# SerezD/gen_adversarial

Hardware: AMD Instinct MI355X
Metric: purified images/sec (attack+encode+decode) (higher is better)
Workload: dtype f32 storage; contractions as 3x bf16 MFMA (hi/lo split), fp32 accumulate; 1 GPU; configs[1]: NVAE purify + VGG-11, 64x64, PGD-Linf step (fwd + input-grad), bs 256 images/GPU x EoT 32 = 8192 defender rows per step, alphas ours_cosine_no_preprocessing_ids.yaml x0.7, assumed NVAE config (C=32, 3x8 groups, 20 latents); images_per_gpu=256, eot=32, rows_per_gpu=8192, chunk_rows=1024, streams=2, parallelism=image-sharded x1

## Files before the change

### gen_adversarial_amd/_lib.py

```python
from __future__ import annotations

import ctypes as C
import os

import torch

_HERE = os.path.dirname(os.path.abspath(__file__))
LIB_PATH = os.environ.get('GA_OPS_LIB') or os.path.join(_HERE, 'libga_ops.so')

GA_ACT_NONE, GA_ACT_SILU, GA_ACT_ELU, GA_ACT_RELU, GA_ACT_LRELU, GA_ACT_FLRELU = 0, 1, 2, 3, 4, 5
GA_CONV_ADDEND_RELU, GA_CONV_ADDEND_PRE_DACT, GA_CONV_PRO_PRELU, GA_CONV_DACT_PRELU = 1, 2, 4, 8
(GA_OP_CONV, GA_OP_DWCONV5, GA_OP_REDUCE, GA_OP_SE_EXCITE, GA_OP_SE_APPLY, GA_OP_BILINEAR_BWD, GA_OP_SAMPLER,
 GA_OP_DML, GA_OP_MAXPOOL, GA_OP_IMAGE_IO, GA_OP_AXPBY, GA_OP_BLUR, GA_OP_REP_SUM, GA_OP_INTERLEAVE2,
 GA_OP_MAXPOOL3S2, GA_OP_AVGPOOL_ACT, GA_OP_GCONV, GA_OP_PRELU, GA_OP_UNARY, GA_OP_MODOUT, GA_OP_UP2_BLUR, GA_OP_PIXELNORM,
 GA_OP_LATENT_MIX, GA_OP_POOL_DENORM, GA_OP_ATTN, GA_OP_LAYERNORM, GA_OP_RESIZE2_CROP, GA_OP_DEC_CELL, GA_OP_AVAE, GA_OP_DEC_CELL_HALO) = range(1, 31)
GA_AVAE_ADAIN, GA_AVAE_AVGPOOL, GA_AVAE_PIXELNORM, GA_AVAE_SAMPLE = 0, 1, 2, 3
ABI_VERSION = 8
ERRORS = {0: 'GA_OK', -1: 'GA_E_BADARG', -2: 'GA_E_ALIGN', -3: 'GA_E_UNSUPPORTED', -4: 'GA_E_LAUNCH'}

fp = C.c_void_p
i32 = C.c_int
f32 = C.c_float


class ConvDesc(C.Structure):
    _fields_ = [('x', fp), ('ldx', i32), ('x2', fp), ('ldx2', i32), ('w', fp), ('bias', fp),
                ('pro_scale', fp), ('pro_shift', fp), ('addend', fp), ('ldadd', i32),
                ('addend2', fp), ('ldadd2', i32), ('dact_x', fp), ('lddact', i32),
                ('dact_scale', fp), ('dact_shift', fp), ('y', fp), ('ldy', i32),
                ('N', i32), ('Hi', i32), ('Wi', i32), ('C1', i32), ('C2', i32),
                ('Ho', i32), ('Wo', i32), ('Cout', i32),
                ('KH', i32), ('KW', i32), ('sn', i32), ('sd', i32), ('pad', i32),
                ('pro_act', i32), ('pro_per_row', i32), ('dact_act', i32), ('addend_bcast_n', i32), ('tile', i32),
                ('splits', i32), ('ws', fp), ('ws_floats', C.c_long),
                ('x_bytes', C.c_uint), ('x2_bytes', C.c_uint), ('w_bytes', C.c_uint), ('dact_rep', i32),
                ('w_hi', fp), ('w_lo', fp), ('addend_rep', i32), ('flags', i32), ('w_frag', fp)]


class DwDesc(C.Structure):
    _fields_ = [('x', fp), ('w', fp), ('bias', fp), ('dact_x', fp), ('y', fp),
                ('N', i32), ('H', i32), ('W', i32), ('C', i32),
                ('pro_act', i32), ('dact_act', i32), ('up2', i32), ('pool2', i32), ('act_rep', i32), ('_reserved', i32)]


class ReduceDesc(C.Structure):
    _fields_ = [('a', fp), ('b', fp), ('out', fp), ('N', i32), ('P', i32), ('C', i32), ('scale', f32),
                ('ws', fp), ('ws_floats', C.c_long), ('gate', fp), ('skip', fp), ('scaled', fp), ('a_src', fp), ('a_w', fp)]


class SeExciteDesc(C.Structure):
    _fields_ = [('m', fp), ('w1', fp), ('b1', fp), ('w2', fp), ('b2', fp), ('hid', fp), ('gate', fp),
                ('dgate', fp), ('pro_scale', fp), ('pro_shift', fp),
                ('N', i32), ('C', i32), ('Hd', i32), ('P', i32), ('res_scale', f32), ('backward', i32),
                ('t', fp), ('dout', fp), ('skip', fp), ('out', fp), ('act_rep', i32), ('_reserved', i32)]


class SeApplyDesc(C.Structure):
    _fields_ = [('skip', fp), ('t', fp), ('gate', fp), ('out', fp),
                ('N', i32), ('H', i32), ('W', i32), ('C', i32), ('skip_mode', i32), ('res_scale', f32)]


class BilinearBwdDesc(C.Structure):
    _fields_ = [('dhigh', fp), ('dlow', fp), ('N', i32), ('h', i32), ('w', i32), ('C', i32), ('accumulate', i32)]


class SamplerDesc(C.Structure):
    _fields_ = [('mu_q', fp), ('ldq', i32), ('p', fp), ('ldp', i32), ('eps', fp), ('eps_nchw', i32),
                ('z', fp), ('dz', fp), ('dmu_q', fp), ('dp', fp),
                ('N', i32), ('h', i32), ('w', i32), ('NL', i32),
                ('alpha', f32), ('one_minus_alpha', f32), ('temp', f32), ('backward', i32),
                ('q_rep', i32), ('dmu_q_rows', fp), ('ldz', i32), ('act_rep', i32), ('mode', i32), ('_reserved', i32),
                ('alpha_rows', fp), ('alpha_ld', i32), ('alpha_col', i32)]


class DmlDesc(C.Structure):
    _fields_ = [('logits', fp), ('ld', i32), ('nmix', i32), ('img_nchw', fp), ('img_nhwc', fp),
                ('dimg_nhwc', fp), ('dimg_nchw', fp), ('dlogits', fp),
                ('N', i32), ('H', i32), ('W', i32), ('backward', i32), ('ld_img', i32), ('act_rep', i32)]


class MaxpoolDesc(C.Structure):
    _fields_ = [('x', fp), ('y', fp), ('dy', fp), ('dx', fp), ('N', i32), ('H', i32), ('W', i32), ('C', i32),
                ('backward', i32), ('act_rep', i32)]


class ImageIoDesc(C.Structure):
    _fields_ = [('x_nchw', fp), ('noise_nchw', fp), ('noise_coef', fp), ('y_nhwc', fp), ('dy_nhwc', fp),
                ('dx_nchw', fp), ('N', i32), ('C', i32), ('H', i32), ('W', i32), ('rep', i32), ('backward', i32),
                ('ld', i32), ('s2d', i32), ('cot_rep', i32), ('_reserved', i32)]


class AxpbyDesc(C.Structure):
    _fields_ = [('x', fp), ('y', fp), ('n', C.c_long), ('alpha', f32), ('beta', f32)]


class BlurDesc(C.Structure):
    _fields_ = [('x', fp), ('y', fp), ('taps', fp), ('planes', i32), ('H', i32), ('W', i32), ('k', i32), ('backward', i32),
                ('radius', i32), ('tmp', fp)]


class RepSumDesc(C.Structure):
    _fields_ = [('x', fp), ('y', fp), ('rows', C.c_long), ('inner', C.c_long), ('rep', i32), ('accumulate', i32)]


class Interleave2Desc(C.Structure):
    _fields_ = [('s', fp * 4), ('y', fp), ('dact_x', fp), ('dact_scale', fp), ('dact_shift', fp), ('addend', fp),
                ('addend2', fp), ('N', i32), ('H', i32), ('W', i32), ('C', i32), ('dact_act', i32), ('dact_prelu', i32),
                ('lds', i32), ('dact_rep', i32)]


class Maxpool3s2Desc(C.Structure):
    _fields_ = [('x', fp), ('y', fp), ('dy', fp), ('dx', fp), ('N', i32), ('H', i32), ('W', i32), ('C', i32),
                ('backward', i32)]


class AvgpoolActDesc(C.Structure):
    _fields_ = [('x', fp), ('y', fp), ('dy', fp), ('dx', fp), ('N', i32), ('P', i32), ('C', i32), ('act', i32),
                ('backward', i32), ('_reserved', i32)]


class GconvDesc(C.Structure):
    _fields_ = [('x', fp), ('w', fp), ('bias', fp), ('dact_x', fp), ('y', fp),
                ('N', i32), ('Hi', i32), ('Wi', i32), ('Ho', i32), ('Wo', i32), ('C', i32), ('cg', i32),
                ('KH', i32), ('KW', i32), ('stride', i32), ('pad', i32), ('pro_act', i32), ('dact_act', i32), ('_reserved', i32)]


class PreluDesc(C.Structure):
    _fields_ = [('x', fp), ('slope', fp), ('y', fp), ('dy', fp), ('dx', fp), ('rows', C.c_long), ('C', i32), ('backward', i32)]


class UnaryDesc(C.Structure):
    _fields_ = [('x', fp), ('g', fp), ('y', fp), ('n', C.c_long), ('mode', i32), ('eps', f32)]


class ModoutDesc(C.Structure):
    _fields_ = [('t', fp), ('scale', fp), ('add', fp), ('out', fp), ('dout', fp), ('dt', fp),
                ('N', i32), ('P', i32), ('C', i32), ('act', i32), ('backward', i32), ('W', i32), ('dt_planes', fp * 4),
                ('ld_planes', i32), ('_reserved2', i32), ('red', fp), ('ws', fp), ('ws_floats', C.c_long), ('t_planes', fp * 4)]


class Up2BlurDesc(C.Structure):
    _fields_ = [('lo_in', fp), ('hi', fp), ('hi_in', fp), ('lo', fp), ('N', i32), ('H', i32), ('W', i32), ('C', i32),
                ('backward', i32), ('_reserved', i32)]


class PixelnormDesc(C.Structure):
    _fields_ = [('x', fp), ('y', fp), ('rows', C.c_long), ('C', i32)]


class LatentMixDesc(C.Structure):
    _fields_ = [('codes', fp), ('avg', fp), ('styles', fp), ('alpha', fp), ('out', fp), ('dout', fp), ('dcodes', fp),
                ('R', i32), ('J', i32), ('D', i32), ('backward', i32), ('rep', i32), ('alpha_ld', i32)]


class PoolDenormDesc(C.Structure):
    _fields_ = [('x', fp), ('y', fp), ('dy', fp), ('dx', fp), ('N', i32), ('H', i32), ('W', i32), ('k', i32), ('ld', i32),
                ('backward', i32), ('dy_nchw', fp), ('band', i32), ('_reserved', i32)]


class AttnDesc(C.Structure):
    _fields_ = [('q', fp), ('k', fp), ('v', fp), ('out', fp), ('p', fp), ('dout', fp), ('ds', fp), ('dq', fp), ('dk', fp), ('dv', fp),
                ('ldq', i32), ('ldk', i32), ('ldv', i32), ('ldo', i32), ('lddq', i32), ('lddk', i32), ('lddv', i32),
                ('N', i32), ('Tq', i32), ('Tk', i32), ('heads', i32), ('dh', i32), ('scale', f32), ('backward', i32)]


class LayernormDesc(C.Structure):
    _fields_ = [('a', fp), ('b', fp), ('gamma', fp), ('beta', fp), ('y', fp), ('stats', fp), ('dy', fp), ('dx', fp),
                ('rows', C.c_long), ('C', i32), ('eps', f32), ('backward', i32), ('accumulate', i32)]


class Resize2CropDesc(C.Structure):
    _fields_ = [('x', fp), ('y', fp), ('dy', fp), ('dx', fp), ('N', i32), ('H', i32), ('W', i32), ('C', i32), ('crop', i32),
                ('backward', i32), ('accumulate', i32), ('_reserved', i32)]


class DecCellDesc(C.Structure):
    _fields_ = [('x', fp), ('w1_hi', fp), ('w1_lo', fp), ('b1', fp), ('wd', fp), ('wd_bwd', fp), ('bd', fp),
                ('w2_hi', fp), ('w2_lo', fp), ('b2', fp), ('dout', fp), ('pro_scale', fp), ('pro_shift', fp), ('y', fp),
                ('N', i32), ('H', i32), ('W', i32), ('C', i32), ('Hd', i32), ('backward', i32), ('act_rep', i32), ('variant', i32)]


class DecCellHaloDesc(C.Structure):
    _fields_ = [('x', fp), ('w1_hi', fp), ('w1_lo', fp), ('b1', fp), ('wd', fp), ('wd_bwd', fp), ('bd', fp),
                ('w2_hi', fp), ('w2_lo', fp), ('b2', fp), ('w1t_hi', fp), ('w1t_lo', fp), ('dout', fp), ('pro_scale', fp), ('pro_shift', fp),
                ('addend', fp), ('addend2', fp), ('y', fp),
                ('N', i32), ('H', i32), ('W', i32), ('Cin', i32), ('Cout', i32), ('Hd', i32), ('backward', i32), ('up', i32)]


class AvaeDesc(C.Structure):
    _fields_ = [('x', fp), ('a', fp), ('b', fp), ('c', fp), ('s', fp), ('dy', fp), ('y', fp), ('y2', fp),
                ('mode', i32), ('backward', i32), ('N', i32), ('P', i32), ('C', i32), ('k', i32), ('H', i32), ('W', i32),
                ('f0', f32), ('_reserved', i32)]


class _OpUnion(C.Union):
    _fields_ = [('conv', ConvDesc), ('dw', DwDesc), ('red', ReduceDesc), ('se', SeExciteDesc), ('app', SeApplyDesc),
                ('bil', BilinearBwdDesc), ('smp', SamplerDesc), ('dml', DmlDesc), ('mp', MaxpoolDesc),
                ('io', ImageIoDesc), ('ax', AxpbyDesc), ('blur', BlurDesc), ('rs', RepSumDesc), ('il', Interleave2Desc),
                ('mp3', Maxpool3s2Desc), ('ap', AvgpoolActDesc), ('gc', GconvDesc), ('pr', PreluDesc), ('un', UnaryDesc), ('mo', ModoutDesc), ('ub', Up2BlurDesc), ('lm', LatentMixDesc),
                ('pd', PoolDenormDesc), ('at', AttnDesc), ('ln', LayernormDesc), ('rc', Resize2CropDesc), ('dc', DecCellDesc), ('pn', PixelnormDesc), ('av', AvaeDesc), ('dh', DecCellHaloDesc)]


class Op(C.Structure):
    _fields_ = [('kind', i32), ('_pad', i32), ('u', _OpUnion)]


_KIND_FIELD = {GA_OP_CONV: 'conv', GA_OP_DWCONV5: 'dw', GA_OP_REDUCE: 'red', GA_OP_SE_EXCITE: 'se',
               GA_OP_SE_APPLY: 'app', GA_OP_BILINEAR_BWD: 'bil', GA_OP_SAMPLER: 'smp', GA_OP_DML: 'dml',
               GA_OP_MAXPOOL: 'mp', GA_OP_IMAGE_IO: 'io', GA_OP_AXPBY: 'ax', GA_OP_BLUR: 'blur', GA_OP_REP_SUM: 'rs',
               GA_OP_INTERLEAVE2: 'il', GA_OP_MAXPOOL3S2: 'mp3', GA_OP_AVGPOOL_ACT: 'ap', GA_OP_GCONV: 'gc', GA_OP_PRELU: 'pr', GA_OP_UNARY: 'un', GA_OP_MODOUT: 'mo', GA_OP_UP2_BLUR: 'ub', GA_OP_PIXELNORM: 'pn',
               GA_OP_LATENT_MIX: 'lm', GA_OP_POOL_DENORM: 'pd', GA_OP_ATTN: 'at', GA_OP_LAYERNORM: 'ln', GA_OP_RESIZE2_CROP: 'rc', GA_OP_DEC_CELL: 'dc', GA_OP_AVAE: 'av', GA_OP_DEC_CELL_HALO: 'dh'}
_DESC_KIND = {ConvDesc: GA_OP_CONV, DwDesc: GA_OP_DWCONV5, ReduceDesc: GA_OP_REDUCE, SeExciteDesc: GA_OP_SE_EXCITE,
              SeApplyDesc: GA_OP_SE_APPLY, BilinearBwdDesc: GA_OP_BILINEAR_BWD, SamplerDesc: GA_OP_SAMPLER,
              DmlDesc: GA_OP_DML, MaxpoolDesc: GA_OP_MAXPOOL, ImageIoDesc: GA_OP_IMAGE_IO, AxpbyDesc: GA_OP_AXPBY,
              BlurDesc: GA_OP_BLUR, RepSumDesc: GA_OP_REP_SUM, Interleave2Desc: GA_OP_INTERLEAVE2,
              Maxpool3s2Desc: GA_OP_MAXPOOL3S2, AvgpoolActDesc: GA_OP_AVGPOOL_ACT, GconvDesc: GA_OP_GCONV,
              PreluDesc: GA_OP_PRELU, UnaryDesc: GA_OP_UNARY, ModoutDesc: GA_OP_MODOUT, Up2BlurDesc: GA_OP_UP2_BLUR,
              PixelnormDesc: GA_OP_PIXELNORM, LatentMixDesc: GA_OP_LATENT_MIX, PoolDenormDesc: GA_OP_POOL_DENORM,
              AttnDesc: GA_OP_ATTN, LayernormDesc: GA_OP_LAYERNORM, Resize2CropDesc: GA_OP_RESIZE2_CROP, DecCellDesc: GA_OP_DEC_CELL, AvaeDesc: GA_OP_AVAE, DecCellHaloDesc: GA_OP_DEC_CELL_HALO}

EXPORTS = ['ga_conv2d', 'ga_dwconv5', 'ga_rowchan_reduce', 'ga_se_excite', 'ga_se_apply', 'ga_bilinear_up2_bwd',
           'ga_sampler_mix', 'ga_dml_mean', 'ga_maxpool2', 'ga_image_io', 'ga_axpby', 'ga_plan_run', 'ga_plan_time',
           'ga_plan_profile', 'ga_split_bf16', 'ga_gauss_blur', 'ga_rep_sum', 'ga_interleave2', 'ga_maxpool3s2', 'ga_avgpool_act', 'ga_gconv', 'ga_prelu', 'ga_unary', 'ga_modout', 'ga_up2_blur', 'ga_pixelnorm', 'ga_latent_mix', 'ga_pool_denorm', 'ga_attn', 'ga_layernorm', 'ga_resize2_crop', 'ga_dec_cell', 'ga_dec_cell_supported', 'ga_dec_cell_halo', 'ga_dec_cell_halo_supported', 'ga_avae', 'ga_microbench_hbm_copy', 'ga_microbench_mfma_bf16', 'ga_microbench_mfma_bf16_shape', 'ga_graph_capture', 'ga_graph_launch', 'ga_graph_destroy',
           'ga_last_hip_error', 'ga_abi_version', 'ga_sizeof_op', 'ga_debug_set_conv_row_limit']


def _load():
    if not os.path.exists(LIB_PATH):
        raise ImportError(f'{LIB_PATH} is missing: build it with `python -c "import __graft_entry__ as g; g.build()"` '
                          f'or `make -C gen_adversarial_amd/csrc` — there is no CPU fallback on the product path')
    lib = C.CDLL(LIB_PATH)
    for n, d in (('ga_conv2d', ConvDesc), ('ga_dwconv5', DwDesc), ('ga_rowchan_reduce', ReduceDesc),
                 ('ga_se_excite', SeExciteDesc), ('ga_se_apply', SeApplyDesc), ('ga_bilinear_up2_bwd', BilinearBwdDesc),
                 ('ga_sampler_mix', SamplerDesc), ('ga_dml_mean', DmlDesc), ('ga_maxpool2', MaxpoolDesc),
                 ('ga_image_io', ImageIoDesc), ('ga_gauss_blur', BlurDesc), ('ga_interleave2', Interleave2Desc),
                 ('ga_maxpool3s2', Maxpool3s2Desc), ('ga_avgpool_act', AvgpoolActDesc), ('ga_gconv', GconvDesc), ('ga_prelu', PreluDesc),
                 ('ga_unary', UnaryDesc), ('ga_modout', ModoutDesc), ('ga_up2_blur', Up2BlurDesc),
                 ('ga_latent_mix', LatentMixDesc), ('ga_pool_denorm', PoolDenormDesc), ('ga_attn', AttnDesc),
                 ('ga_layernorm', LayernormDesc), ('ga_resize2_crop', Resize2CropDesc), ('ga_dec_cell', DecCellDesc), ('ga_avae', AvaeDesc), ('ga_dec_cell_halo', DecCellHaloDesc)):
        f = getattr(lib, n)
        f.argtypes = [C.POINTER(d), C.c_void_p]
        f.restype = C.c_int
    lib.ga_axpby.argtypes = [fp, fp, C.c_long, f32, f32, C.c_void_p]
    lib.ga_axpby.restype = C.c_int
    lib.ga_plan_run.argtypes = [C.POINTER(Op), C.c_int, C.c_void_p, C.POINTER(C.c_int)]
    lib.ga_plan_run.restype = C.c_int
    lib.ga_plan_time.argtypes = [C.POINTER(Op), C.c_int, C.c_void_p, C.c_int, C.POINTER(f32), C.POINTER(f32),
                                 C.POINTER(C.c_long)]
    lib.ga_plan_time.restype = C.c_int
    lib.ga_plan_profile.argtypes = [C.POINTER(Op), C.c_int, C.c_void_p, C.POINTER(f32)]
    lib.ga_plan_profile.restype = C.c_int
    lib.ga_rep_sum.argtypes = [fp, fp, C.c_long, C.c_long, C.c_int, C.c_int, C.c_void_p]
    lib.ga_rep_sum.restype = C.c_int
    lib.ga_pixelnorm.argtypes = [fp, fp, C.c_long, C.c_int, C.c_void_p]
    lib.ga_pixelnorm.restype = C.c_int
    lib.ga_graph_capture.argtypes = [C.POINTER(Op), C.c_int, C.c_void_p, C.POINTER(C.c_void_p)]
    lib.ga_graph_capture.restype = C.c_int
    lib.ga_graph_launch.argtypes = [C.c_void_p, C.c_void_p]
    lib.ga_graph_launch.restype = C.c_int
    lib.ga_graph_destroy.argtypes = [C.c_void_p]
    lib.ga_graph_destroy.restype = C.c_int
    lib.ga_split_bf16.argtypes = [fp, fp, fp, C.c_long, C.c_void_p]
    lib.ga_split_bf16.restype = C.c_int
    lib.ga_last_hip_error.restype = C.c_char_p
    lib.ga_abi_version.restype = C.c_int
    lib.ga_sizeof_op.restype = C.c_ulong
    lib.ga_debug_set_conv_row_limit.restype = C.c_long
    lib.ga_dec_cell_supported.argtypes = [C.c_int] * 5
    lib.ga_dec_cell_supported.restype = C.c_int
    lib.ga_dec_cell_halo_supported.argtypes = [C.c_int] * 5
    lib.ga_dec_cell_halo_supported.restype = C.c_int
    lib.ga_debug_set_conv_row_limit.argtypes = [C.c_long]
    lib.ga_microbench_hbm_copy.argtypes = [fp, fp, C.c_long, C.c_void_p]
    lib.ga_microbench_hbm_copy.restype = C.c_int
    lib.ga_microbench_mfma_bf16.argtypes = [fp, C.c_int, C.c_int, C.c_void_p]
    lib.ga_microbench_mfma_bf16.restype = C.c_int
    lib.ga_microbench_mfma_bf16_shape.argtypes = [fp, C.c_int, C.c_int, C.c_int, C.c_void_p]
    lib.ga_microbench_mfma_bf16_shape.restype = C.c_int
    if lib.ga_abi_version() != ABI_VERSION:
        raise ImportError(f'ABI mismatch: {LIB_PATH} reports GA_ABI_VERSION {lib.ga_abi_version()}, the binding is written for '
                          f'{ABI_VERSION}: rebuild with `make -C gen_adversarial_amd/csrc`')
    if lib.ga_sizeof_op() != C.sizeof(Op):
        raise ImportError(f'ABI mismatch: library ga_op is {lib.ga_sizeof_op()} bytes, binding is {C.sizeof(Op)}')
    return lib


lib = _load()


class GaError(RuntimeError):
    pass


def check(rc: int, what: str = ''):
    if rc != 0:
        extra = f' ({lib.ga_last_hip_error().decode()})' if rc == -4 else ''
        raise GaError(f'{what}: {ERRORS.get(rc, rc)}{extra}')


def make_op(desc) -> Op:
    op = Op()
    op.kind = _DESC_KIND[type(desc)]
    setattr(op.u, _KIND_FIELD[op.kind], desc)
    return op


_DIRECT = {ConvDesc: 'ga_conv2d', DwDesc: 'ga_dwconv5', ReduceDesc: 'ga_rowchan_reduce', SeExciteDesc: 'ga_se_excite',
           SeApplyDesc: 'ga_se_apply', BilinearBwdDesc: 'ga_bilinear_up2_bwd', SamplerDesc: 'ga_sampler_mix',
           DmlDesc: 'ga_dml_mean', MaxpoolDesc: 'ga_maxpool2', ImageIoDesc: 'ga_image_io', BlurDesc: 'ga_gauss_blur',
           Interleave2Desc: 'ga_interleave2', Maxpool3s2Desc: 'ga_maxpool3s2', AvgpoolActDesc: 'ga_avgpool_act',
           GconvDesc: 'ga_gconv', PreluDesc: 'ga_prelu', UnaryDesc: 'ga_unary', ModoutDesc: 'ga_modout', Up2BlurDesc: 'ga_up2_blur',
           LatentMixDesc: 'ga_latent_mix', PoolDenormDesc: 'ga_pool_denorm', AttnDesc: 'ga_attn', LayernormDesc: 'ga_layernorm',
           Resize2CropDesc: 'ga_resize2_crop', DecCellDesc: 'ga_dec_cell', AvaeDesc: 'ga_avae', DecCellHaloDesc: 'ga_dec_cell_halo'}


def run(desc, stream: int = 0):
    if isinstance(desc, AxpbyDesc):
        check(lib.ga_axpby(desc.x, desc.y, desc.n, desc.alpha, desc.beta, stream), 'ga_axpby')
        return
    if isinstance(desc, PixelnormDesc):
        check(lib.ga_pixelnorm(desc.x, desc.y, desc.rows, desc.C, stream), 'ga_pixelnorm')
        return
    if isinstance(desc, RepSumDesc):
        check(lib.ga_rep_sum(desc.x, desc.y, desc.rows, desc.inner, desc.rep, desc.accumulate, stream), 'ga_rep_sum')
        return
    name = _DIRECT[type(desc)]
    check(getattr(lib, name)(C.byref(desc), stream), name)


class Plan:

    def __init__(self):
        self.descs = []
        self.names = []
        self._arr = None

    def add(self, desc, name: str = ''):
        self.descs.append(desc)
        self.names.append(name)
        self._arr = None

    def finalize(self):
        arr = (Op * len(self.descs))()
        for i, d in enumerate(self.descs):
            arr[i] = make_op(d)
        self._arr = arr
        return self

    def __len__(self):
        return len(self.descs)

    def run(self, stream: int = 0, start: int = 0, end: int = None):
        if self._arr is None:
            self.finalize()
        end = len(self.descs) if end is None else end
        if end <= start:
            return
        failed = C.c_int(-1)
        first = C.cast(C.byref(self._arr, start * C.sizeof(Op)), C.POINTER(Op))
        rc = lib.ga_plan_run(first, end - start, stream, C.byref(failed))
        if rc != 0:
            check(rc, f'plan op #{start + failed.value} ({self.names[start + failed.value]})')

    def capture(self, stream: int):
        if self._arr is None:
            self.finalize()
        h = C.c_void_p()
        check(lib.ga_graph_capture(self._arr, len(self.descs), stream, C.byref(h)), 'ga_graph_capture')
        return h

    @staticmethod
    def launch_graph(handle, stream: int):
        check(lib.ga_graph_launch(handle, stream), 'ga_graph_launch')

    @staticmethod
    def destroy_graph(handle):
        lib.ga_graph_destroy(handle)

    def profile(self, stream: int = 0):
        if self._arr is None:
            self.finalize()
        out = (f32 * len(self.descs))()
        check(lib.ga_plan_profile(self._arr, len(self.descs), stream, out), 'ga_plan_profile')
        return list(out)

    def time(self, stream: int = 0, iters: int = 1, per_conv: bool = False):
        if self._arr is None:
            self.finalize()
        total, conv, nconv = f32(0), f32(0), C.c_long(0)
        rc = lib.ga_plan_time(self._arr, len(self.descs), stream, iters, C.byref(total),
                              C.byref(conv) if per_conv else None, C.byref(nconv) if per_conv else None)
        check(rc, 'ga_plan_time')
        return total.value, conv.value, nconv.value
```

### gen_adversarial_amd/csrc/conv_epilogue.h

```cpp
#pragma once
#include "ga_common.h"

namespace ga {

__device__ __forceinline__ size_t dact_row(const ga_conv_desc& d, const size_t m, const int HoWo) {
    if (d.dact_rep <= 1) return m;
    const size_t n = m / (size_t)HoWo;
    return (n / (size_t)d.dact_rep) * (size_t)HoWo + (m - n * (size_t)HoWo);
}

__device__ __forceinline__ void epilogue4(const ga_conv_desc& d, const int m, const int co, floatx4 v, const int HoWo) {
    if (d.bias) v += *reinterpret_cast<const floatx4*>(d.bias + co);
    if ((d.flags & GA_CONV_ADDEND_PRE_DACT) && d.addend) v += *reinterpret_cast<const floatx4*>(d.addend + (size_t)m * d.ldadd + co);
    if (d.dact_x) {
        floatx4 u = *reinterpret_cast<const floatx4*>(d.dact_x + dact_row(d, (size_t)m, HoWo) * d.lddact + co);
        floatx4 ds = {1.f, 1.f, 1.f, 1.f};
        if (d.flags & GA_CONV_DACT_PRELU) {
            ds = *reinterpret_cast<const floatx4*>(d.dact_scale + co);
#pragma unroll
            for (int e = 0; e < 4; ++e) v[e] *= u[e] > 0.f ? 1.f : ds[e];
        } else {
            if (d.dact_scale) {
                ds = *reinterpret_cast<const floatx4*>(d.dact_scale + co);
                u = u * ds + *reinterpret_cast<const floatx4*>(d.dact_shift + co);
            }
#pragma unroll
            for (int e = 0; e < 4; ++e) v[e] *= act_bwd_fast(u[e], d.dact_act) * ds[e];
        }
    }
    if (d.addend && !(d.flags & GA_CONV_ADDEND_PRE_DACT)) {
        size_t am = d.addend_bcast_n ? (size_t)(m % HoWo) : (size_t)m;
        if (d.addend_rep > 1) am = (size_t)((m / HoWo) / d.addend_rep) * HoWo + (m % HoWo);
        floatx4 a = *reinterpret_cast<const floatx4*>(d.addend + am * d.ldadd + co);
        if (d.flags & GA_CONV_ADDEND_RELU) { for (int e = 0; e < 4; ++e) a[e] = fmaxf(a[e], 0.f); }
        v += a;
    }
    if (d.addend2) v += *reinterpret_cast<const floatx4*>(d.addend2 + (size_t)m * d.ldadd2 + co);
    *reinterpret_cast<floatx4*>(d.y + (size_t)m * d.ldy + co) = v;
}

__device__ __forceinline__ void epilogue1(const ga_conv_desc& d, const int m, const int co, float v, const int HoWo) {
    if (d.bias) v += d.bias[co];
    if ((d.flags & GA_CONV_ADDEND_PRE_DACT) && d.addend) v += d.addend[(size_t)m * d.ldadd + co];
    if (d.dact_x) {
        float ds = 1.f, db = 0.f;
        if (d.dact_scale) { ds = d.dact_scale[co]; db = d.dact_shift[co]; }
        if (d.flags & GA_CONV_DACT_PRELU) {
            v *= d.dact_x[dact_row(d, (size_t)m, HoWo) * d.lddact + co] > 0.f ? 1.f : ds;
        } else {
            const float u = d.dact_x[dact_row(d, (size_t)m, HoWo) * d.lddact + co] * ds + db;
            v *= act_bwd_fast(u, d.dact_act) * ds;
        }
    }
    if (d.addend && !(d.flags & GA_CONV_ADDEND_PRE_DACT)) {
        size_t am = d.addend_bcast_n ? (size_t)(m % HoWo) : (size_t)m;
        if (d.addend_rep > 1) am = (size_t)((m / HoWo) / d.addend_rep) * HoWo + (m % HoWo);
        const float a = d.addend[am * d.ldadd + co];
        v += (d.flags & GA_CONV_ADDEND_RELU) ? fmaxf(a, 0.f) : a;
    }
    if (d.addend2) v += d.addend2[(size_t)m * d.ldadd2 + co];
    d.y[(size_t)m * d.ldy + co] = v;
}


template <int TM, int TN, class F>
__device__ __forceinline__ void acc_walk(floatx16 (&acc)[TM][TN], const int lane, F&& f) {
    const int lrow = lane & 31, lh = lane >> 5;
#pragma unroll
    for (int i = 0; i < TM; ++i)
#pragma unroll
        for (int j = 0; j < TN; ++j)
#pragma unroll
            for (int r = 0; r < 16; ++r) f(i * 32 + (r & 3) + 8 * (r >> 2) + 4 * lh, j * 32 + lrow, acc[i][j][r]);
}
template <int TM2, int TN2, class F>
__device__ __forceinline__ void acc_walk(floatx4 (&acc)[TM2][TN2], const int lane, F&& f) {
    const int lc = lane & 15, lq = lane >> 4;
#pragma unroll
    for (int i = 0; i < TM2; ++i)
#pragma unroll
        for (int j = 0; j < TN2; ++j)
#pragma unroll
            for (int r = 0; r < 4; ++r) f(i * 16 + 4 * lq + r, j * 16 + lc, acc[i][j][r]);
}

template <int WM, int WN, int TM, int TN, class ACC>
__device__ __forceinline__ void conv_epilogue(const ga_conv_desc& d, ACC& acc, float* smem, const int m0,
                                              const int n0, const int M, const int vec_out, const int splits, const int split,
                                              const int tw_shift = 31, const int row_stride = 0) {
    const int tw_mask = (int)((1u << tw_shift) - 1u);
    auto mrow = [&](const int r) __attribute__((always_inline)) { return m0 + (r >> tw_shift) * row_stride + (r & tw_mask); };
    constexpr int BM = WM * TM * 32, BN = WN * TN * 32;
    constexpr int LDC = BN + 4;
    const int tid = threadIdx.x, lane = tid & 63, wave = tid >> 6;
    const int wm = wave / WN, wn = wave % WN;
    const int HoWo = d.Ho * d.Wo;
    float* ws = splits > 1 ? d.ws + (size_t)split * M * d.Cout : nullptr;
    if (vec_out) {
        float* Cs = smem;
        constexpr int QL = BN / 4;
        constexpr int ROWS = 256 / QL;
        constexpr int NB = (BM / ROWS) < 4 ? (BM / ROWS) : 4;
        constexpr int NIT = BM / (ROWS * NB);
        static_assert(NIT * ROWS * NB == BM, "whole batches");
        const int q = tid % QL, rr = tid / QL;
        const int co = n0 + 4 * q;
        const bool mine = co < d.Cout;
        floatx4 u[1][NB], a1[1][NB], a2[1][NB];
        auto issue = [&](const int set, const int rb0) __attribute__((always_inline)) {
#pragma unroll
            for (int k = 0; k < NB; ++k) {
                const int r = rb0 + k * ROWS;
                const int mr = mrow(r);
                const bool ok = mr < M;
                if (d.dact_x) {
                    const size_t m = ok ? dact_row(d, (size_t)mr, HoWo) : 0;
                    u[set][k] = *reinterpret_cast<const floatx4*>(d.dact_x + m * d.lddact + co);
                }
                if (d.addend) {
                    size_t m = ok ? (size_t)mr : 0;
                    if (d.addend_bcast_n) m = m % HoWo;
                    if (d.addend_rep > 1) m = ((m / HoWo) / d.addend_rep) * HoWo + (m % HoWo);
                    a1[set][k] = *reinterpret_cast<const floatx4*>(d.addend + m * d.ldadd + co);
                }
                if (d.addend2) {
                    const size_t m = ok ? (size_t)mr : 0;
                    a2[set][k] = *reinterpret_cast<const floatx4*>(d.addend2 + m * d.ldadd2 + co);
                }
            }
        };
        floatx4 bias4 = {0.f, 0.f, 0.f, 0.f}, ds4 = {1.f, 1.f, 1.f, 1.f}, dt4 = {0.f, 0.f, 0.f, 0.f};
        if (mine && !ws) {
            if (d.bias) bias4 = *reinterpret_cast<const floatx4*>(d.bias + co);
            if (d.dact_x && d.dact_scale) {
                ds4 = *reinterpret_cast<const floatx4*>(d.dact_scale + co);
                dt4 = *reinterpret_cast<const floatx4*>(d.dact_shift + co);
            }
        }
        acc_walk(acc, lane, [&](const int row, const int col, const float v) {
            Cs[(wm * TM * 32 + row) * LDC + wn * TN * 32 + col] = v;
        });
        __syncthreads();
        if (mine) {
#pragma unroll 1
            for (int it = 0; it < NIT; ++it) {
                const int rb0 = rr + it * ROWS * NB, set = 0;
                floatx4 v[NB];
                bool ok[NB];
                if (!ws) issue(0, rb0);
#pragma unroll
                for (int k = 0; k < NB; ++k) {
                    const int r = rb0 + k * ROWS;
                    ok[k] = mrow(r) < M;
                    v[k] = *reinterpret_cast<const floatx4*>(Cs + r * LDC + 4 * q);
                }
                if (ws) {
#pragma unroll
                    for (int k = 0; k < NB; ++k)
                        if (ok[k]) *reinterpret_cast<floatx4*>(ws + (size_t)mrow(rb0 + k * ROWS) * d.Cout + co) = v[k];
                    continue;
                }
#pragma unroll
                for (int k = 0; k < NB; ++k) {
                    floatx4 o = v[k] + bias4;
                    const bool pre = (d.flags & GA_CONV_ADDEND_PRE_DACT) != 0;
                    if (pre && d.addend) o += a1[set][k];
                    if (d.dact_x && (d.flags & GA_CONV_DACT_PRELU)) {
#pragma unroll
                        for (int e = 0; e < 4; ++e) o[e] *= u[set][k][e] > 0.f ? 1.f : ds4[e];
                    } else if (d.dact_x) {
                        const floatx4 uu = u[set][k] * ds4 + dt4;
                        if (d.dact_act == GA_ACT_SILU) {
#pragma unroll
                            for (int e = 0; e < 4; ++e) { const float sg = fast_sigmoid(uu[e]); o[e] *= sg * (1.0f + uu[e] * (1.0f - sg)) * ds4[e]; }
                        } else {
#pragma unroll
                            for (int e = 0; e < 4; ++e) o[e] *= act_bwd_fast(uu[e], d.dact_act) * ds4[e];
                        }
                    }
                    if (d.addend && !pre) {
                        if (d.flags & GA_CONV_ADDEND_RELU) {
#pragma unroll
                            for (int e = 0; e < 4; ++e) o[e] += fmaxf(a1[set][k][e], 0.f);
                        } else {
                            o += a1[set][k];
                        }
                    }
                    if (d.addend2) o += a2[set][k];
                    if (ok[k]) *reinterpret_cast<floatx4*>(d.y + (size_t)mrow(rb0 + k * ROWS) * d.ldy + co) = o;
                }
            }
        }
    } else {
        acc_walk(acc, lane, [&](const int row, const int col, const float v) {
            const int co = n0 + wn * TN * 32 + col, m = mrow(wm * TM * 32 + row);
            if (co < d.Cout && m < M) {
                if (ws) ws[(size_t)m * d.Cout + co] = v;
                else epilogue1(d, m, co, v, HoWo);
            }
        });
    }
}

}
```

### gen_adversarial_amd/csrc/conv_mfma.hip

```cpp
#include "ga_common.h"
#include "conv_epilogue.h"

namespace ga {

constexpr int BK = 32;
constexpr int LDK = 36;

template <int WM, int WN, int TM, int TN, bool VEC, int PRO, bool FAST>
__global__ void __launch_bounds__(256)
conv_mfma_kernel(const ga_conv_desc d, const int tilesN, const int M, const int Ctot, const int Ktot, const int nkc,
                 const int vec_out, const fastdiv fd_howo, const fastdiv fd_wo) {
    constexpr int BM = WM * TM * 32, BN = WN * TN * 32;
    constexpr int RA = BM / 32, RB = BN / 32;
    constexpr int LDC = BN + 4;
    extern __shared__ __attribute__((aligned(16))) float smem[];
    float* As = smem;
    float* Bs = smem + 2 * BM * LDK;

    int bid;
    {
        const int nb = gridDim.x, orig = blockIdx.x;
        const int q = nb >> 3, r = nb & 7, xcd = orig & 7, k = orig >> 3;
        bid = (xcd < r ? xcd * (q + 1) : r * (q + 1) + (xcd - r) * q) + k;
    }
// ... 244 lines not shown
            }
#pragma unroll
            for (int i = 0; i < RB; ++i)
                *reinterpret_cast<floatx4*>(Bb + (r0 + 32 * i) * LDK + 4 * c4) = (okmask >> (16 + i)) & 1u ? rb[i] : zero;
        } else {
#pragma unroll
            for (int i = 0; i < RA; ++i) *reinterpret_cast<floatx4*>(Ab + (r0 + 32 * i) * LDK + 4 * c4) = ra[i];
#pragma unroll
            for (int i = 0; i < RB; ++i) *reinterpret_cast<floatx4*>(Bb + (r0 + 32 * i) * LDK + 4 * c4) = rb[i];
        }
    };

    floatx16 acc[TM][TN];
#pragma unroll
    for (int i = 0; i < TM; ++i)
#pragma unroll
        for (int j = 0; j < TN; ++j)
#pragma unroll
            for (int r = 0; r < 16; ++r) acc[i][j][r] = 0.f;

    const int T = d.KH * d.KW * nkc;
    const int splits = gridDim.y, split = blockIdx.y;
    const int tper = (T + splits - 1) / splits;
    const int t_begin = split * tper;
    const int t_end = min(T, t_begin + tper);

    const int lrow = lane & 31, lh = lane >> 5;
    if (t_begin < t_end) {
        seek_tile(t_begin);
        issue_tile(t_begin);
        finish_tile(0);
    }
    __syncthreads();
    for (int t = t_begin; t < t_end; ++t) {
        const int buf = (t - t_begin) & 1;
        if (t + 1 < t_end) issue_tile(t + 1);
        const float* Ab = As + buf * BM * LDK + (wm * TM * 32 + lrow) * LDK + 4 * lh;
        const float* Bb = Bs + buf * BN * LDK + (wn * TN * 32 + lrow) * LDK + 4 * lh;
#pragma unroll
        for (int kk = 0; kk < BK / 8; ++kk) {
            floatx4 af[TM], bf[TN];
#pragma unroll
            for (int i = 0; i < TM; ++i) af[i] = *reinterpret_cast<const floatx4*>(Ab + i * 32 * LDK + kk * 8);
#pragma unroll
            for (int j = 0; j < TN; ++j) bf[j] = *reinterpret_cast<const floatx4*>(Bb + j * 32 * LDK + kk * 8);
#pragma unroll
            for (int s = 0; s < 4; ++s)
#pragma unroll
                for (int i = 0; i < TM; ++i)
#pragma unroll
                    for (int j = 0; j < TN; ++j)
                        acc[i][j] = __builtin_amdgcn_mfma_f32_32x32x2f32(af[i][s], bf[j][s], acc[i][j], 0, 0, 0);
        }
        if (t + 1 < t_end) finish_tile(buf ^ 1);
        __syncthreads();
    }

    conv_epilogue<WM, WN, TM, TN>(d, acc, smem, m0, n0, M, vec_out, splits, split);
}

__global__ void __launch_bounds__(256) conv_splitk_reduce_kernel(const ga_conv_desc d, const int M, const int splits, const int vec_out) {
    const int HoWo = d.Ho * d.Wo;
    const size_t slab = (size_t)M * d.Cout;
    if (vec_out) {
        const long total4 = (long)slab / 4;
        const int C4 = d.Cout / 4;
        for (long i = (long)blockIdx.x * 256 + threadIdx.x; i < total4; i += (long)gridDim.x * 256) {
            floatx4 v = *reinterpret_cast<const floatx4*>(d.ws + i * 4);
            for (int s = 1; s < splits; ++s) v += *reinterpret_cast<const floatx4*>(d.ws + s * slab + i * 4);
            epilogue4(d, (int)(i / C4), (int)(i % C4) * 4, v, HoWo);
        }
    } else {
        for (long i = (long)blockIdx.x * 256 + threadIdx.x; i < (long)slab; i += (long)gridDim.x * 256) {
            float v = d.ws[i];
            for (int s = 1; s < splits; ++s) v += d.ws[s * slab + i];
            epilogue1(d, (int)(i / d.Cout), (int)(i % d.Cout), v, HoWo);
        }
    }
}

template <int WM, int WN, int TM, int TN, bool VEC, int PRO, bool FAST>
static void launch_inst(const ga_conv_desc& d, hipStream_t stream, dim3 grid, size_t lds, int tilesN, int M, int Ctot,
                        int Ktot, int nkc, int vec_out) {
    static dyn_lds_cache attr;
    (void)ensure_dyn_lds(attr, reinterpret_cast<const void*>(&conv_mfma_kernel<WM, WN, TM, TN, VEC, PRO, FAST>), lds);
    hipLaunchKernelGGL((conv_mfma_kernel<WM, WN, TM, TN, VEC, PRO, FAST>), grid, dim3(256), lds, stream, d, tilesN, M, Ctot, Ktot, nkc, vec_out,
                       make_fastdiv(d.Ho * d.Wo), make_fastdiv(d.Wo));
}

template <int WM, int WN, int TM, int TN>
static int launch_conv(const ga_conv_desc& d, hipStream_t stream, bool vec, int vec_out, int splits) {
    constexpr int BM = WM * TM * 32, BN = WN * TN * 32;
    const int M = d.N * d.Ho * d.Wo;
    const int Ctot = d.C1 + d.C2;
    const int Ktot = d.KH * d.KW * Ctot;
    const int nkc = (Ctot + BK - 1) / BK;
    const int tilesM = (M + BM - 1) / BM, tilesN = (d.Cout + BN - 1) / BN;
    size_t lds = (size_t)2 * (BM + BN) * LDK * sizeof(float);
    const size_t lds_c = (size_t)BM * (BN + 4) * sizeof(float);
    if (lds_c > lds) lds = lds_c;
    const dim3 grid(tilesM * tilesN, splits);
    const int pro = d.pro_scale && d.pro_per_row ? 2 : ((d.pro_scale || d.pro_act) ? 1 : 0);
    const bool fast = vec && d.sd == 1 && (d.C2 == 0 || d.C1 % BK == 0) && d.KH * d.KW <= 32 &&
                      d.x_bytes > 0 && d.w_bytes > 0 && (d.C2 == 0 || d.x2_bytes > 0);
    if (fast) {
        if (pro == 0) launch_inst<WM, WN, TM, TN, true, 0, true>(d, stream, grid, lds, tilesN, M, Ctot, Ktot, nkc, vec_out);
        else if (pro == 1) launch_inst<WM, WN, TM, TN, true, 1, true>(d, stream, grid, lds, tilesN, M, Ctot, Ktot, nkc, vec_out);
        else launch_inst<WM, WN, TM, TN, true, 2, true>(d, stream, grid, lds, tilesN, M, Ctot, Ktot, nkc, vec_out);
    } else if (vec) {
        if (pro == 0) launch_inst<WM, WN, TM, TN, true, 0, false>(d, stream, grid, lds, tilesN, M, Ctot, Ktot, nkc, vec_out);
        else if (pro == 1) launch_inst<WM, WN, TM, TN, true, 1, false>(d, stream, grid, lds, tilesN, M, Ctot, Ktot, nkc, vec_out);
        else launch_inst<WM, WN, TM, TN, true, 2, false>(d, stream, grid, lds, tilesN, M, Ctot, Ktot, nkc, vec_out);
    } else {
        launch_inst<WM, WN, TM, TN, false, 1, false>(d, stream, grid, lds, tilesN, M, Ctot, Ktot, nkc, vec_out);
    }
    return check_launch();
}

int conv_bf3_dispatch(const ga_conv_desc& d, hipStream_t stream, int tile, int vec_out, int splits);
int conv_bf3_supports(const ga_conv_desc& d);
int conv_halo3_dispatch(const ga_conv_desc& d, hipStream_t stream, int tile, int vec_out, int splits);
int conv_halo3_supports(const ga_conv_desc& d);
int conv_thin3_dispatch(const ga_conv_desc& d, hipStream_t stream, int vec_out, int splits);
int conv_thin3_supports(const ga_conv_desc& d);

}

static long g_conv_row_limit = 0x7fffff00L;
static long ga_conv_row_limit() { return g_conv_row_limit; }
extern "C" long ga_debug_set_conv_row_limit(long bytes) {
    const long old = g_conv_row_limit;
    g_conv_row_limit = bytes > 0 ? bytes : 0x7fffff00L;
    return old;
}

extern "C" int ga_conv2d(const ga_conv_desc* dp, void* stream_) {
    ga::clear_stale_error();
    using namespace ga;
    if (!dp) return GA_E_BADARG;
    const ga_conv_desc& d = *dp;
    hipStream_t stream = reinterpret_cast<hipStream_t>(stream_);
    if (!d.x || !d.w || !d.y) return GA_E_BADARG;
    if (d.N <= 0 || d.Hi <= 0 || d.Wi <= 0 || d.C1 <= 0 || d.C2 < 0 || d.Ho <= 0 || d.Wo <= 0 || d.Cout <= 0) return GA_E_BADARG;
    if (d.KH <= 0 || d.KW <= 0 || d.sn <= 0 || d.sd <= 0 || d.pad < 0) return GA_E_BADARG;
    if (d.sd & (d.sd - 1)) return GA_E_UNSUPPORTED;
    if (d.C2 > 0 && !d.x2) return GA_E_BADARG;
    if ((d.pro_scale == nullptr) != (d.pro_shift == nullptr)) return GA_E_BADARG;
    if (d.dact_x && ((d.dact_scale == nullptr) != (d.dact_shift == nullptr))) return GA_E_BADARG;
    if (d.ldx < d.C1 || (d.C2 > 0 && d.ldx2 < d.C2) || d.ldy < d.Cout) return GA_E_BADARG;
    if (d.addend && d.ldadd < d.Cout) return GA_E_BADARG;
    if (d.addend2 && d.ldadd2 < d.Cout) return GA_E_BADARG;
    if (d.dact_x && d.lddact < d.Cout) return GA_E_BADARG;
    if (d.dact_x && d.dact_rep > 1 && d.N % d.dact_rep) return GA_E_BADARG;
    {
        const long row_x = (long)d.Hi * d.Wi * d.ldx * 4, row_x2 = d.C2 > 0 ? (long)d.Hi * d.Wi * d.ldx2 * 4 : 0;
        long row_max = row_x > row_x2 ? row_x : row_x2;
        const long pix_out = (long)d.Ho * d.Wo * 4;
        if (pix_out * d.ldy > row_max) row_max = pix_out * d.ldy;
        if (d.addend && !d.addend_bcast_n && pix_out * d.ldadd > row_max) row_max = pix_out * d.ldadd;
        if (d.addend2 && pix_out * d.ldadd2 > row_max) row_max = pix_out * d.ldadd2;
        if (d.dact_x && pix_out * d.lddact > row_max) row_max = pix_out * d.lddact;
        const long lim = ga_conv_row_limit();
        if (d.N > 1 && row_max * d.N >= lim && row_max < lim) {
            int sub = (int)((lim - 1) / row_max);
            const int arep = d.addend && !d.addend_bcast_n && d.addend_rep > 1 ? d.addend_rep : 1;
            const int drep = d.dact_x && d.dact_rep > 1 ? d.dact_rep : 1;
            if (arep > 1 || drep > 1) {
                const long both = (long)arep * drep;
                if (d.N % arep || d.N % drep) return GA_E_BADARG;
                sub -= (int)(sub % both);
                if (sub < both) return GA_E_UNSUPPORTED;
            }
            for (int n0 = 0; n0 < d.N; n0 += sub) {
                ga_conv_desc s = d;
                s.N = d.N - n0 < sub ? d.N - n0 : sub;
                const size_t pin = (size_t)n0 * d.Hi * d.Wi, pout = (size_t)n0 * d.Ho * d.Wo;
                s.x = d.x + pin * d.ldx;
                if (d.x2) s.x2 = d.x2 + pin * d.ldx2;
                s.y = d.y + pout * d.ldy;
                if (d.addend && !d.addend_bcast_n) s.addend = d.addend + (size_t)(n0 / arep) * d.Ho * d.Wo * d.ldadd;
                if (d.addend2) s.addend2 = d.addend2 + pout * d.ldadd2;
                if (d.dact_x) s.dact_x = d.dact_x + (size_t)(n0 / drep) * d.Ho * d.Wo * d.lddact;
                if (d.pro_scale && d.pro_per_row) {
                    s.pro_scale = d.pro_scale + (size_t)n0 * d.C1;
                    s.pro_shift = d.pro_shift + (size_t)n0 * d.C1;
                }
                const int rc = ga_conv2d(&s, stream_);
                if (rc != GA_OK) return rc;
            }
            return GA_OK;
        }
    }
    if ((long)d.N * d.Ho * d.Wo > 0x7fffffffL) return GA_E_UNSUPPORTED;
    if ((long)d.KH * d.KW * (d.C1 + d.C2) > 0x7fffffffL) return GA_E_UNSUPPORTED;
    const long M = (long)d.N * d.Ho * d.Wo;
    int splits = d.splits <= 1 ? 1 : d.splits;
    if (splits > 1) {
        if (!d.ws || d.ws_floats < (long)splits * M * d.Cout) return GA_E_BADARG;
        const int T = d.KH * d.KW * ((d.C1 + d.C2 + 31) / 32);
        if (splits > T) splits = T;
        if (splits > 65535) return GA_E_UNSUPPORTED;
    }

    const bool vec = (d.C1 % 4 == 0) && (d.C2 % 4 == 0) && (d.ldx % 4 == 0) && (d.C2 == 0 || d.ldx2 % 4 == 0) &&
                     aligned16(d.x) && aligned16(d.w) && (d.C2 == 0 || aligned16(d.x2)) &&
                     (!d.pro_scale || (aligned16(d.pro_scale) && aligned16(d.pro_shift)));
    const bool vec_out = (d.Cout % 4 == 0) && (d.ldy % 4 == 0) && aligned16(d.y) && (!d.bias || aligned16(d.bias)) &&
                         (!d.addend || (d.ldadd % 4 == 0 && aligned16(d.addend))) &&
                         (!d.addend2 || (d.ldadd2 % 4 == 0 && aligned16(d.addend2))) &&
                         (!d.dact_x || (d.lddact % 4 == 0 && aligned16(d.dact_x) &&
                                        (!d.dact_scale || (aligned16(d.dact_scale) && aligned16(d.dact_shift))))) &&
                         (splits == 1 || aligned16(d.ws));

    int tile = d.tile;
    if (tile == 0) {
        if (d.Cout <= 32) tile = 4;
        else if (d.Cout <= 64) tile = (M >= 128 * 256) ? 2 : 3;
        else {
            const long b128 = ((M + 127) / 128) * ((d.Cout + 127) / 128);
            const long b12864 = ((M + 127) / 128) * ((d.Cout + 63) / 64);
            if (b128 >= 512) tile = 1;
            else if (b12864 >= 512) tile = 2;
            else tile = 3;
        }
    }
    ga_conv_desc k = d;
    const long xb = ((long)d.N * d.Hi * d.Wi - 1) * d.ldx * 4 + (long)d.C1 * 4;
    const long x2b = d.C2 > 0 ? ((long)d.N * d.Hi * d.Wi - 1) * d.ldx2 * 4 + (long)d.C2 * 4 : 0;
    const long wb = (long)d.Cout * d.KH * d.KW * (d.C1 + d.C2) * 4;
    const long lim = 0x7fffff00L;
    k.x_bytes = xb < lim ? (unsigned)xb : 0;
    k.x2_bytes = x2b < lim ? (unsigned)x2b : 0;
    k.w_bytes = wb < lim ? (unsigned)wb : 0;
    const int Ctot = d.C1 + d.C2;
    const bool bf3 = d.w_hi && d.w_lo && vec && d.sd == 1 && (d.C2 == 0 || d.C1 % 32 == 0) && (Ctot % 8 == 0) &&
                     d.KH * d.KW <= 32 && k.x_bytes > 0 && k.w_bytes > 0 && (d.C2 == 0 || k.x2_bytes > 0) &&
                     aligned16(d.w_hi) && aligned16(d.w_lo) && conv_bf3_supports(d);
    int rc;
    if (tile == 11) {
        if (!(bf3 && vec_out && conv_thin3_supports(d))) return GA_E_UNSUPPORTED;
        rc = conv_thin3_dispatch(k, stream, vec_out, splits);
    } else if (tile >= 5 && tile <= 10) {
        if (!(bf3 && vec_out && conv_halo3_supports(d))) return GA_E_UNSUPPORTED;
        rc = conv_halo3_dispatch(k, stream, tile, vec_out, splits);
    } else if (bf3) {
        rc = conv_bf3_dispatch(k, stream, tile, vec_out, splits);
    } else {
        switch (tile) {
            case 1: rc = launch_conv<2, 2, 2, 2>(k, stream, vec, vec_out, splits); break;
            case 2: rc = launch_conv<4, 1, 1, 2>(k, stream, vec, vec_out, splits); break;
            case 3: rc = launch_conv<2, 2, 1, 1>(k, stream, vec, vec_out, splits); break;
            case 4: rc = launch_conv<4, 1, 1, 1>(k, stream, vec, vec_out, splits); break;
            default: return GA_E_UNSUPPORTED;
        }
    }
    if (rc != GA_OK || splits == 1) return rc;
    long items = M * d.Cout / (vec_out ? 4 : 1);
    long blocks = (items + 255) / 256;
    if (blocks > 4096) blocks = 4096;
    hipLaunchKernelGGL(conv_splitk_reduce_kernel, dim3((unsigned)blocks), dim3(256), 0, stream, k, (int)M, splits, vec_out);
    return check_launch();
}
```

### gen_adversarial_amd/csrc/elementwise.hip

```cpp
#include "ga_common.h"

namespace ga {

struct reduce_a_src {
    const float* a; const float* src; floatx4 w0, w1, w2, w3; int C;
    __device__ __forceinline__ reduce_a_src(const ga_rowchan_reduce_desc& d, const int n, const int c) : C(d.C) {
        a = d.a ? d.a + (size_t)n * d.P * d.C + c : nullptr;
        src = d.a ? nullptr : d.a_src + (size_t)n * d.P * 4;
        if (!d.a) {
            w0 = *reinterpret_cast<const floatx4*>(d.a_w + (size_t)(c + 0) * 4); w1 = *reinterpret_cast<const floatx4*>(d.a_w + (size_t)(c + 1) * 4);
            w2 = *reinterpret_cast<const floatx4*>(d.a_w + (size_t)(c + 2) * 4); w3 = *reinterpret_cast<const floatx4*>(d.a_w + (size_t)(c + 3) * 4);
        }
    }
    __device__ __forceinline__ floatx4 operator()(const int p) const {
        if (a) return *reinterpret_cast<const floatx4*>(a + (size_t)p * C);
        const floatx4 s = *reinterpret_cast<const floatx4*>(src + (size_t)p * 4);
        floatx4 v;
        v[0] = w0[0] * s[0] + w0[1] * s[1] + w0[2] * s[2] + w0[3] * s[3];
        v[1] = w1[0] * s[0] + w1[1] * s[1] + w1[2] * s[2] + w1[3] * s[3];
        v[2] = w2[0] * s[0] + w2[1] * s[1] + w2[2] * s[2] + w2[3] * s[3];
        v[3] = w3[0] * s[0] + w3[1] * s[1] + w3[2] * s[2] + w3[3] * s[3];
        return v;
    }
};

__device__ __forceinline__ void reduce_scaled_store(const ga_rowchan_reduce_desc& d, const floatx4 gt, const size_t o, const floatx4 a) {
    floatx4 sk = {0.f, 0.f, 0.f, 0.f}, r;
    if (d.skip) sk = *reinterpret_cast<const floatx4*>(d.skip + o);
#pragma unroll
    for (int e = 0; e < 4; ++e) r[e] = __builtin_fmaf(gt[e], a[e], sk[e]);
    *reinterpret_cast<floatx4*>(d.scaled + o) = r;
}

__global__ void __launch_bounds__(256) rowchan_reduce_kernel(const ga_rowchan_reduce_desc d, const int nchunks) {
    __shared__ floatx4 part[16][16];
    const int tid = threadIdx.x, c4 = tid & 15, pl = tid >> 4;
    const int n = blockIdx.x / nchunks, chunk = blockIdx.x % nchunks;
    const int c = chunk * 64 + 4 * c4;
    floatx4 acc = {0.f, 0.f, 0.f, 0.f};
    if (c < d.C) {
        const reduce_a_src a(d, n, c);
        const float* b = d.b ? d.b + (size_t)n * d.P * d.C + c : nullptr;
        if (d.scaled) {
            const floatx4 gt = *reinterpret_cast<const floatx4*>(d.gate + (size_t)n * d.C + c);
#pragma unroll 4
            for (int p = pl; p < d.P; p += 16) {
                floatx4 v = a(p);
                reduce_scaled_store(d, gt, ((size_t)n * d.P + p) * d.C + c, v);
                if (b) v *= *reinterpret_cast<const floatx4*>(b + (size_t)p * d.C);
                acc += v;
            }
        } else {
#pragma unroll 8
            for (int p = pl; p < d.P; p += 16) {
                floatx4 v = a(p);
                if (b) v *= *reinterpret_cast<const floatx4*>(b + (size_t)p * d.C);
                acc += v;
            }
        }
    }
    part[pl][c4] = acc;
    __syncthreads();
    if (pl == 0 && c < d.C) {
        floatx4 s = part[0][c4];
#pragma unroll
        for (int i = 1; i < 16; ++i) s += part[i][c4];
        *reinterpret_cast<floatx4*>(d.out + (size_t)n * d.C + c) = s * d.scale;
    }
}

__global__ void __launch_bounds__(256) rowchan_reduce_split_kernel(const ga_rowchan_reduce_desc d, const int nchunks, const int ql,
                                                                   const int S, const int seg_len) {
    __shared__ floatx4 part[256];
    const int tid = threadIdx.x, c4 = tid % ql, pl = tid / ql, PL = 256 / ql;
    int bi = blockIdx.x;
    const int seg = bi % S; bi /= S;
    const int chunk = bi % nchunks, n = bi / nchunks;
    const int c = chunk * 64 + 4 * c4;
    floatx4 acc = {0.f, 0.f, 0.f, 0.f};
    if (c < d.C) {
        const reduce_a_src a(d, n, c);
        const float* b = d.b ? d.b + (size_t)n * d.P * d.C + c : nullptr;
        const int p1 = min(d.P, (seg + 1) * seg_len);
        if (d.scaled) {
            const floatx4 gt = *reinterpret_cast<const floatx4*>(d.gate + (size_t)n * d.C + c);
#pragma unroll 4
            for (int p = seg * seg_len + pl; p < p1; p += PL) {
                floatx4 v = a(p);
                reduce_scaled_store(d, gt, ((size_t)n * d.P + p) * d.C + c, v);
                if (b) v *= *reinterpret_cast<const floatx4*>(b + (size_t)p * d.C);
                acc += v;
            }
        } else {
#pragma unroll 8
            for (int p = seg * seg_len + pl; p < p1; p += PL) {
                floatx4 v = a(p);
                if (b) v *= *reinterpret_cast<const floatx4*>(b + (size_t)p * d.C);
                acc += v;
            }
        }
    }
    part[tid] = acc;
    __syncthreads();
    for (int st = PL >> 1; st > 0; st >>= 1) {
        if (pl < st) part[tid] += part[tid + st * ql];
        __syncthreads();
    }
    if (pl == 0 && c < d.C) *reinterpret_cast<floatx4*>(d.ws + ((size_t)n * S + seg) * d.C + c) = part[tid];
}

__global__ void __launch_bounds__(256) rowchan_reduce_final_kernel(const ga_rowchan_reduce_desc d, const int S) {
    const long i = (long)blockIdx.x * 256 + threadIdx.x;
    if (i >= (long)d.N * d.C) return;
    const long n = i / d.C; const int c = (int)(i % d.C);
    float acc = 0.f;
    for (int sgm = 0; sgm < S; ++sgm) acc += d.ws[((size_t)n * S + sgm) * d.C + c];
    d.out[i] = acc * d.scale;
}

__device__ __forceinline__ floatx4 se_merge_expr(const floatx4 s, const float rs, const floatx4 g, const floatx4 t) {
    floatx4 o;
#pragma unroll
    for (int e = 0; e < 4; ++e) o[e] = __builtin_fmaf(rs * g[e], t[e], s[e]);
    return o;
}

__global__ void __launch_bounds__(256) se_excite_kernel(const ga_se_excite_desc d) {
    extern __shared__ __attribute__((aligned(16))) float sm[];
    float* s_in = sm;
    float* s_hid = sm + d.C;
    float* s_part = sm + ((d.C + d.Hd + 3) & ~3);
    const int n = blockIdx.x, tid = threadIdx.x;
    const int na = (d.backward && d.act_rep > 1) ? n / d.act_rep : n;
    if (d.t) {
        const int C4 = d.C >> 2, PL = 256 / C4;
        const int q = tid % C4, pl = tid / C4;
        if (pl < PL) {
            floatx4 acc = {0.f, 0.f, 0.f, 0.f};
            const float* a = d.t + (size_t)na * d.P * d.C + 4 * q;
            const float* b = d.backward ? d.dout + (size_t)n * d.P * d.C + 4 * q : nullptr;
#pragma unroll 8
            for (int p = pl; p < d.P; p += PL) {
                floatx4 v = *reinterpret_cast<const floatx4*>(a + (size_t)p * d.C);
                if (b) v *= *reinterpret_cast<const floatx4*>(b + (size_t)p * d.C);
                acc += v;
            }
            *reinterpret_cast<floatx4*>(s_part + pl * d.C + 4 * q) = acc;
        }
        __syncthreads();
        const float sc = d.backward ? d.res_scale : 1.0f / (float)d.P;
        for (int c = tid; c < d.C; c += 256) {
            float s = s_part[c];
            for (int k = 1; k < PL; ++k) s += s_part[k * d.C + c];
            s_in[c] = s * sc;
        }
        __syncthreads();
    }
    const int C4 = d.C >> 2;
    int chunks = 256 / d.Hd;
    if (chunks > C4) chunks = C4;
    const int per = (C4 + chunks - 1) / chunks;
    float* s_red = s_part;
    if (!d.backward) {
        if (!d.t) {
            for (int c = tid; c < d.C; c += 256) s_in[c] = d.m[(size_t)n * d.C + c];
            __syncthreads();
        }
        {
            const int j = tid / chunks, ch = tid % chunks;
            if (j < d.Hd) {
                float acc = 0.f;
                const int q0 = ch * per, q1 = min(C4, q0 + per);
                if ((d.C & 3) == 0) {
#pragma unroll 8
                    for (int q = q0; q < q1; ++q) {
                        const floatx4 w = *reinterpret_cast<const floatx4*>(d.w1 + (size_t)j * d.C + 4 * q);
                        const floatx4 v = *reinterpret_cast<const floatx4*>(s_in + 4 * q);
                        acc += w[0] * v[0] + w[1] * v[1] + w[2] * v[2] + w[3] * v[3];
                    }
                }
                s_red[j * chunks + ch] = acc;
            }
        }
        __syncthreads();
        if (tid < d.Hd) {
            float h = d.b1[tid];
            for (int k = 0; k < chunks; ++k) h += s_red[tid * chunks + k];
            if (d.C & 3) {
                h = d.b1[tid];
                for (int c = 0; c < d.C; ++c) h += d.w1[(size_t)tid * d.C + c] * s_in[c];
            }
            s_hid[tid] = h;
            d.hid[(size_t)n * d.Hd + tid] = h;
        }
        __syncthreads();
        for (int c = tid; c < d.C; c += 256) {
            float acc = d.b2[c];
            const float* w = d.w2 + (size_t)c * d.Hd;
            if ((d.Hd & 3) == 0) {
#pragma unroll 8
                for (int j = 0; j < d.Hd; j += 4) {
                    const floatx4 wv = *reinterpret_cast<const floatx4*>(w + j);
                    acc += wv[0] * fmaxf(s_hid[j], 0.f) + wv[1] * fmaxf(s_hid[j + 1], 0.f) +
                           wv[2] * fmaxf(s_hid[j + 2], 0.f) + wv[3] * fmaxf(s_hid[j + 3], 0.f);
                }
            } else {
                for (int j = 0; j < d.Hd; ++j) acc += w[j] * fmaxf(s_hid[j], 0.f);
            }
            const float gv = sigmoidf_(acc);
            d.gate[(size_t)n * d.C + c] = gv;
            if (d.out) s_part[c] = gv;
        }
        if (d.out) {
            __syncthreads();
            const int C4m = d.C >> 2;
            const float* tb = d.t + (size_t)n * d.P * d.C;
            const float* sb = d.skip ? d.skip + (size_t)n * d.P * d.C : nullptr;
            float* ob = d.out + (size_t)n * d.P * d.C;
#pragma unroll 4
            for (int i = tid; i < d.P * C4m; i += 256) {
                const int q = i % C4m;
                const floatx4 t = *reinterpret_cast<const floatx4*>(tb + (size_t)i * 4);
                const floatx4 g = *reinterpret_cast<const floatx4*>(s_part + 4 * q);
                const floatx4 s = sb ? *reinterpret_cast<const floatx4*>(sb + (size_t)i * 4) : floatx4{0.f, 0.f, 0.f, 0.f};
                *reinterpret_cast<floatx4*>(ob + (size_t)i * 4) = se_merge_expr(s, d.res_scale, g, t);
            }
        }
    } else {
        for (int c = tid; c < d.C; c += 256) {
            const float g = d.gate[(size_t)na * d.C + c];
            const float dg = d.t ? s_in[c] : d.dgate[(size_t)n * d.C + c];
            s_in[c] = dg * g * (1.f - g);
        }
        __syncthreads();
        if (256 % d.Hd == 0) {
            const int j = tid % d.Hd, nch = 256 / d.Hd, ch = tid / d.Hd;
            float acc = 0.f;
#pragma unroll 16
            for (int c = ch; c < d.C; c += nch) acc += d.w2[(size_t)c * d.Hd + j] * s_in[c];
            s_red[j * nch + ch] = acc;
            __syncthreads();
            if (tid < d.Hd) {
                float a2 = 0.f;
                for (int k = 0; k < nch; ++k) a2 += s_red[tid * nch + k];
                s_hid[tid] = d.hid[(size_t)na * d.Hd + tid] > 0.f ? a2 : 0.f;
            }
        } else {
            if (tid < d.Hd) {
                float a2 = 0.f;
                for (int c = 0; c < d.C; ++c) a2 += d.w2[(size_t)c * d.Hd + tid] * s_in[c];
                s_hid[tid] = d.hid[(size_t)na * d.Hd + tid] > 0.f ? a2 : 0.f;
            }
        }
        __syncthreads();
        const float invP = 1.0f / (float)d.P;
        for (int c = tid; c < d.C; c += 256) {
            float acc = 0.f;
#pragma unroll 16
            for (int j = 0; j < d.Hd; ++j) acc += d.w1[(size_t)j * d.C + c] * s_hid[j];
            d.pro_scale[(size_t)n * d.C + c] = d.res_scale * d.gate[(size_t)na * d.C + c];
            d.pro_shift[(size_t)n * d.C + c] = acc * invP;
        }
    }
}

__device__ __forceinline__ void bil_src(const int o, const int in, const int out, int& i0, int& i1, float& l1) {
    const float scale = out > 1 ? (float)(in - 1) / (float)(out - 1) : 0.f;
    const float src = scale * (float)o;
    i0 = (int)src;
    i1 = i0 + (i0 < in - 1 ? 1 : 0);
    l1 = src - (float)i0;
}

__global__ void __launch_bounds__(256) se_apply_kernel(const ga_se_apply_desc d, const long total4) {
    const int C4 = d.C / 4;
    for (long i = (long)blockIdx.x * 256 + threadIdx.x; i < total4; i += (long)gridDim.x * 256) {
        const int c4 = (int)(i % C4); long p = i / C4;
        const int w = (int)(p % d.W); p /= d.W;
        const int h = (int)(p % d.H); const int n = (int)(p / d.H);
        const int c = 4 * c4;
        const floatx4 t = *reinterpret_cast<const floatx4*>(d.t + i * 4);
        const floatx4 g = *reinterpret_cast<const floatx4*>(d.gate + (size_t)n * d.C + c);
        floatx4 s;
        if (d.skip_mode == 0) {
            s = d.skip ? *reinterpret_cast<const floatx4*>(d.skip + i * 4) : floatx4{0.f, 0.f, 0.f, 0.f};
        } else if (d.skip_mode == 2) {
            s = *reinterpret_cast<const floatx4*>(d.skip + (((size_t)n * 2 * d.H + 2 * h) * 2 * d.W + 2 * w) * d.C + c);
        } else {
            const int hl = d.H / 2, wl = d.W / 2;
            int h0, h1, w0, w1; float lh, lw;
            bil_src(h, hl, d.H, h0, h1, lh);
            bil_src(w, wl, d.W, w0, w1, lw);
            const float* base = d.skip + (size_t)n * hl * wl * d.C + c;
            const floatx4 x00 = *reinterpret_cast<const floatx4*>(base + ((size_t)h0 * wl + w0) * d.C);
            const floatx4 x01 = *reinterpret_cast<const floatx4*>(base + ((size_t)h0 * wl + w1) * d.C);
            const floatx4 x10 = *reinterpret_cast<const floatx4*>(base + ((size_t)h1 * wl + w0) * d.C);
            const floatx4 x11 = *reinterpret_cast<const floatx4*>(base + ((size_t)h1 * wl + w1) * d.C);
            const float h0l = 1.f - lh, w0l = 1.f - lw;
            s = h0l * (w0l * x00 + lw * x01) + lh * (w0l * x10 + lw * x11);
        }
        *reinterpret_cast<floatx4*>(d.out + i * 4) = se_merge_expr(s, d.res_scale, g, t);
    }
}

__global__ void __launch_bounds__(256) bilinear_up2_bwd_kernel(const ga_bilinear_up2_bwd_desc d, const long total4) {
    const int C4 = d.C / 4;
    const int H = 2 * d.h, W = 2 * d.w;
    for (long i = (long)blockIdx.x * 256 + threadIdx.x; i < total4; i += (long)gridDim.x * 256) {
        const int c4 = (int)(i % C4); long p = i / C4;
        const int wl = (int)(p % d.w); p /= d.w;
        const int hl = (int)(p % d.h); const int n = (int)(p / d.h);
        floatx4 acc = {0.f, 0.f, 0.f, 0.f};
        const float* base = d.dhigh + (size_t)n * H * W * d.C + 4 * c4;
        const int hlo = max(0, 2 * hl - 2), hhi = min(H - 1, 2 * hl + 4);
        const int wlo = max(0, 2 * wl - 2), whi = min(W - 1, 2 * wl + 4);
        for (int hh = hlo; hh <= hhi; ++hh) {
            int h0, h1; float lh;
            bil_src(hh, d.h, H, h0, h1, lh);
            const float wh = (h0 == hl ? 1.f - lh : 0.f) + (h1 == hl ? lh : 0.f);
            if (wh == 0.f) continue;
            for (int ww = wlo; ww <= whi; ++ww) {
                int w0, w1; float lw;
                bil_src(ww, d.w, W, w0, w1, lw);
                const float wwt = (w0 == wl ? 1.f - lw : 0.f) + (w1 == wl ? lw : 0.f);
                if (wwt == 0.f) continue;
                acc += (wh * wwt) * *reinterpret_cast<const floatx4*>(base + ((size_t)hh * W + ww) * d.C);
            }
        }
        floatx4* o = reinterpret_cast<floatx4*>(d.dlow + i * 4);
        *o = d.accumulate ? (*o + acc) : acc;
    }
}

__device__ __forceinline__ float softclamp5(float x) { return tanhf(x / 5.0f) * 5.0f; }
__device__ __forceinline__ float dsoftclamp5(float x) { const float t = tanhf(x / 5.0f); return 1.0f - t * t; }

__global__ void __launch_bounds__(256) sampler_kernel(const ga_sampler_desc d, const long total) {
    const int hw = d.h * d.w;
    for (long i = (long)blockIdx.x * 256 + threadIdx.x; i < total; i += (long)gridDim.x * 256) {
        const int c = (int)(i % d.NL); const long pix = i / d.NL;
        const int n = (int)(pix / hw), p = (int)(pix % hw);
        const long zi = d.ldz > 0 ? pix * d.ldz + c : i;
        const int na = (d.backward && d.act_rep > 1) ? n / d.act_rep : n;
        const long apix = (long)na * hw + p;
        if (d.mode == 1) {
            const float e1 = d.eps_nchw ? d.eps[((size_t)na * d.NL + c) * hw + p] : d.eps[apix * d.NL + c];
            const float mu_s = d.mu_q[apix * d.ldq + c] + d.p[apix * d.ldp + c];
            const float ls_s = d.mu_q[apix * d.ldq + d.NL + c] + d.p[apix * d.ldp + d.NL + c];
            const float ex = expf(softclamp5(ls_s));
            if (!d.backward) {
                d.z[zi] = softclamp5(mu_s) + (ex + 0.01f) * e1;
            } else {
                const float dz = d.dz[zi];
                const float dmu = dz * dsoftclamp5(mu_s), dls = dz * e1 * ex * dsoftclamp5(ls_s);
                d.dmu_q[pix * d.ldq + c] = dmu;
                d.dmu_q[pix * d.ldq + d.NL + c] = dls;
                d.dp[pix * d.ldp + c] = dmu;
                d.dp[pix * d.ldp + d.NL + c] = dls;
            }
            continue;
        }
        const long qpix = d.q_rep > 1 ? (long)(na / d.q_rep) * hw + p : apix;
        const float mq = d.mu_q[qpix * d.ldq + c];
        const float mp = d.p ? d.p[apix * d.ldp + c] : 0.f;
        const float ls = d.p ? d.p[apix * d.ldp + d.NL + c] : 0.f;
        const float e = d.eps_nchw ? d.eps[((size_t)na * d.NL + c) * hw + p] : d.eps[apix * d.NL + c];
        const float sig = d.temp * expf(softclamp5(ls));
        float a = d.alpha, om = d.one_minus_alpha;
        if (d.alpha_rows) {
            const float* ar = d.alpha_rows + (size_t)na * d.alpha_ld + 2 * d.alpha_col;
            a = ar[0]; om = ar[1];
        }
        if (!d.backward) {
            const float enc_mu = softclamp5(mp + mq);
            const float smp = e * sig + softclamp5(mp);
            d.z[zi] = om * enc_mu + a * smp;
        } else {
            const float dz = d.dz[zi];
            const float denc = om * dz * dsoftclamp5(mp + mq);
            if (d.q_rep > 1) d.dmu_q_rows[d.ldz > 0 ? pix * d.ldq + c : i] = denc; else d.dmu_q[pix * d.ldq + c] = denc;
            if (d.dp) {
                d.dp[pix * d.ldp + c] = denc + a * dz * dsoftclamp5(mp);
                d.dp[pix * d.ldp + d.NL + c] = a * dz * e * sig * dsoftclamp5(ls);
            }
// ... 633 lines not shown
#pragma unroll
                for (int e = 0; e < 4; ++e) v[e] *= u[e] > 0.f ? 1.f : ds[e];
            } else {
                if (d.dact_scale) {
                    ds = *reinterpret_cast<const floatx4*>(d.dact_scale + 4 * q);
                    u = u * ds + *reinterpret_cast<const floatx4*>(d.dact_shift + 4 * q);
                }
#pragma unroll
                for (int e = 0; e < 4; ++e) v[e] *= act_bwd_fast(u[e], d.dact_act) * ds[e];
            }
        }
        if (d.addend) v += *reinterpret_cast<const floatx4*>(d.addend + o);
        if (d.addend2) v += *reinterpret_cast<const floatx4*>(d.addend2 + o);
        *reinterpret_cast<floatx4*>(d.y + o) = v;
    }
}

__device__ __forceinline__ int reflect_idx(int t, const int n) {
    if (t < 0) t = -t;
    if (t >= n) t = 2 * (n - 1) - t;
    return t;
}

__device__ __forceinline__ float blur_tap_sum(const float* line, const int stride, const int n, const int i, const float* g,
                                              const int k, const bool adjoint, const int r) {
    const int p = k / 2;
    float acc = 0.f;
    if (!adjoint) {
        for (int q = p - r; q <= p + r; ++q) acc += g[q] * line[reflect_idx(i + q - p, n) * stride];
    } else {
        for (int q = p - r; q <= p + r; ++q) {
            const int a = i - q + p;
            if (a >= 0 && a < n) acc += g[q] * line[a * stride];
            if (i >= 1) { const int b2 = -i - q + p; if (b2 >= 0 && b2 < n) acc += g[q] * line[b2 * stride]; }
            if (i <= n - 2) { const int c2 = 2 * (n - 1) - i - q + p; if (c2 >= 0 && c2 < n) acc += g[q] * line[c2 * stride]; }
        }
    }
    return acc;
}

__global__ void __launch_bounds__(256) gauss_blur_kernel(const ga_blur_desc d, const int r) {
    extern __shared__ float bl_s[];
    float* a = bl_s;
    float* b = bl_s + d.H * d.W;
    float* g = b + d.H * d.W;
    const int HW = d.H * d.W;
    const float* src = d.x + (size_t)blockIdx.x * HW;
    for (int i = threadIdx.x; i < HW; i += 256) a[i] = src[i];
    for (int i = threadIdx.x; i < d.k; i += 256) g[i] = d.taps[i];
    __syncthreads();
    const bool adj = d.backward != 0;
    for (int i = threadIdx.x; i < HW; i += 256) {
        const int h = i / d.W, w = i - h * d.W;
        b[i] = adj ? blur_tap_sum(a + w, d.W, d.H, h, g, d.k, true, r) : blur_tap_sum(a + h * d.W, 1, d.W, w, g, d.k, false, r);
    }
    __syncthreads();
    float* dst = d.y + (size_t)blockIdx.x * HW;
    for (int i = threadIdx.x; i < HW; i += 256) {
        const int h = i / d.W, w = i - h * d.W;
        dst[i] = adj ? blur_tap_sum(b + h * d.W, 1, d.W, w, g, d.k, true, r) : blur_tap_sum(b + w, d.W, d.H, h, g, d.k, false, r);
    }
}

__global__ void __launch_bounds__(256) gauss_blur_pass_kernel(const float* __restrict__ src, float* __restrict__ dst, const float* __restrict__ taps,
                                                              const int H, const int W, const int k, const int r, const int along_y,
                                                              const int adjoint, const int T, const int tiles) {
    extern __shared__ float bl_s[];
    const int plane = blockIdx.x / tiles, tile = blockIdx.x - plane * tiles;
    const size_t base = (size_t)plane * H * W;
    float* g = bl_s;
    float* a = bl_s + ((k + 3) & ~3);
    for (int i = threadIdx.x; i < k; i += 256) g[i] = taps[i];
    if (!along_y) {
        const int h0 = tile * T, nr = min(T, H - h0);
        for (int i = threadIdx.x; i < nr * W; i += 256) a[i] = src[base + (size_t)h0 * W + i];
        __syncthreads();
        for (int i = threadIdx.x; i < nr * W; i += 256) {
            const int hh = i / W, w = i - hh * W;
            dst[base + (size_t)h0 * W + i] = blur_tap_sum(a + hh * W, 1, W, w, g, k, adjoint != 0, r);
        }
    } else {
        const int w0 = tile * T, nc = min(T, W - w0);
        for (int i = threadIdx.x; i < H * T; i += 256) {
            const int h = i / T, c = i - h * T;
            if (c < nc) a[i] = src[base + (size_t)h * W + w0 + c];
        }
        __syncthreads();
        for (int i = threadIdx.x; i < H * T; i += 256) {
            const int h = i / T, c = i - h * T;
            if (c < nc) dst[base + (size_t)h * W + w0 + c] = blur_tap_sum(a + c, T, H, h, g, k, adjoint != 0, r);
        }
    }
}

__global__ void __launch_bounds__(256) rep_sum_kernel(const float* x, float* y, const long total, const long inner, const int rep,
                                                        const int accumulate) {
    for (long i = (long)blockIdx.x * 256 + threadIdx.x; i < total; i += (long)gridDim.x * 256) {
        const long b = i / inner, j = i - b * inner;
        float acc = accumulate ? y[i] : 0.f;
        for (int r = 0; r < rep; ++r) acc += x[(b * rep + r) * inner + j];
        y[i] = acc;
    }
}

__global__ void __launch_bounds__(256) axpby_kernel(const float* x, float* y, const long n, const float a, const float b) {
    for (long i = (long)blockIdx.x * 256 + threadIdx.x; i < n; i += (long)gridDim.x * 256)
        y[i] = a * x[i] + (b == 0.f ? 0.f : b * y[i]);
}

static inline unsigned grid_for(long items) {
    long b = (items + 255) / 256;
    if (b > 2048 * 4) b = 2048 * 4;
    if (b < 1) b = 1;
    return (unsigned)b;
}

}

using namespace ga;

extern "C" int ga_rowchan_reduce(const ga_rowchan_reduce_desc* d, void* s) {
    ga::clear_stale_error();
    if (!d || (!d->a && !(d->a_src && d->a_w)) || !d->out || d->N <= 0 || d->P <= 0 || d->C <= 0) return GA_E_BADARG;
    if (d->C % 4) return GA_E_UNSUPPORTED;
    if ((d->a && !aligned16(d->a)) || !aligned16(d->out) || (d->b && !aligned16(d->b))) return GA_E_ALIGN;
    if (!d->a && (!aligned16(d->a_src) || !aligned16(d->a_w))) return GA_E_ALIGN;
    if (d->scaled && (!d->gate || !aligned16(d->scaled) || !aligned16(d->gate) || (d->skip && !aligned16(d->skip)))) return GA_E_BADARG;
    const int nchunks = (d->C + 63) / 64;
    if (d->ws && d->P >= 4096 && d->N * nchunks < 1024) {
        if (!aligned16(d->ws)) return GA_E_ALIGN;
        long S = d->ws_floats / ((long)d->N * d->C);
        const long want = 2048 / ((long)d->N * nchunks);
        if (S > want) S = want;
        if (S > (d->P + 1023) / 1024) S = (d->P + 1023) / 1024;
        if (S >= 2) {
            const int q = d->C >= 64 ? 16 : d->C / 4;
            int ql = 1;
            while (ql < q) ql <<= 1;
            const int seg_len = (int)((d->P + S - 1) / S);
            hipLaunchKernelGGL(rowchan_reduce_split_kernel, dim3((unsigned)(d->N * nchunks * S)), dim3(256), 0, (hipStream_t)s, *d,
                               nchunks, ql, (int)S, seg_len);
            const long total = (long)d->N * d->C;
            hipLaunchKernelGGL(rowchan_reduce_final_kernel, dim3((unsigned)((total + 255) / 256)), dim3(256), 0, (hipStream_t)s, *d, (int)S);
            return check_launch();
        }
    }
    hipLaunchKernelGGL(rowchan_reduce_kernel, dim3(d->N * nchunks), dim3(256), 0, (hipStream_t)s, *d, nchunks);
    return check_launch();
}

extern "C" int ga_se_excite(const ga_se_excite_desc* d, void* s) {
    ga::clear_stale_error();
    if (!d || !d->w1 || !d->b1 || !d->w2 || !d->b2 || !d->hid || !d->gate || d->N <= 0 || d->C <= 0 || d->Hd <= 0) return GA_E_BADARG;
    if (!d->backward && !d->m && !d->t) return GA_E_BADARG;
    if (d->backward && ((!d->dgate && !d->t) || !d->pro_scale || !d->pro_shift || d->P <= 0)) return GA_E_BADARG;
    if (d->out && (d->backward || !d->t || !aligned16(d->out) || (d->skip && !aligned16(d->skip)))) return GA_E_BADARG;
    if (d->act_rep > 1 && (!d->backward || !d->t || d->N % d->act_rep)) return GA_E_BADARG;
    size_t lds = (size_t)(d->C + d->Hd + 4 + 256) * sizeof(float);
    if (d->Hd > 256) return GA_E_UNSUPPORTED;
    if (d->t) {
        if (d->P <= 0 || (d->backward && !d->dout)) return GA_E_BADARG;
        if (d->C % 4 || d->C > 1024) return GA_E_UNSUPPORTED;
        if (!aligned16(d->t) || (d->dout && !aligned16(d->dout))) return GA_E_ALIGN;
        const size_t red = (size_t)(256 / (d->C / 4)) * d->C * sizeof(float);
        if (red > 256 * sizeof(float)) lds += red - 256 * sizeof(float);
    }
    if (lds > 64 * 1024) return GA_E_UNSUPPORTED;
    hipLaunchKernelGGL(se_excite_kernel, dim3(d->N), dim3(256), lds, (hipStream_t)s, *d);
    return check_launch();
}

extern "C" int ga_se_apply(const ga_se_apply_desc* d, void* s) {
    ga::clear_stale_error();
    if (!d || !d->t || !d->gate || !d->out || d->N <= 0 || d->H <= 0 || d->W <= 0 || d->C <= 0) return GA_E_BADARG;
    if (!d->skip && d->skip_mode != 0) return GA_E_BADARG;
    if (d->C % 4) return GA_E_UNSUPPORTED;
    if (d->skip_mode == 1 && ((d->H | d->W) & 1)) return GA_E_BADARG;
    if (d->skip_mode < 0 || d->skip_mode > 2) return GA_E_UNSUPPORTED;
    if ((d->skip && !aligned16(d->skip)) || !aligned16(d->t) || !aligned16(d->gate) || !aligned16(d->out)) return GA_E_ALIGN;
    const long total4 = (long)d->N * d->H * d->W * (d->C / 4);
    hipLaunchKernelGGL(se_apply_kernel, dim3(grid_for(total4)), dim3(256), 0, (hipStream_t)s, *d, total4);
    return check_launch();
}

extern "C" int ga_bilinear_up2_bwd(const ga_bilinear_up2_bwd_desc* d, void* s) {
    ga::clear_stale_error();
    if (!d || !d->dhigh || !d->dlow || d->N <= 0 || d->h <= 0 || d->w <= 0 || d->C <= 0) return GA_E_BADARG;
    if (d->C % 4) return GA_E_UNSUPPORTED;
    if (!aligned16(d->dhigh) || !aligned16(d->dlow)) return GA_E_ALIGN;
    const long total4 = (long)d->N * d->h * d->w * (d->C / 4);
    hipLaunchKernelGGL(bilinear_up2_bwd_kernel, dim3(grid_for(total4)), dim3(256), 0, (hipStream_t)s, *d, total4);
    return check_launch();
}

extern "C" int ga_sampler_mix(const ga_sampler_desc* d, void* s) {
    ga::clear_stale_error();
    if (!d || !d->mu_q || !d->eps || d->N <= 0 || d->h <= 0 || d->w <= 0 || d->NL <= 0) return GA_E_BADARG;
    if (d->ldq < d->NL || (d->p && d->ldp < 2 * d->NL)) return GA_E_BADARG;
    if (!d->backward && !d->z) return GA_E_BADARG;
    if (d->backward && (!d->dz || (d->q_rep > 1 ? !d->dmu_q_rows : !d->dmu_q) || (d->p && !d->dp))) return GA_E_BADARG;
    if (d->q_rep > 1 && d->N % d->q_rep) return GA_E_BADARG;
    if (d->act_rep > 1 && (!d->backward || d->N % d->act_rep || (d->q_rep > 1 && (d->N / d->act_rep) % d->q_rep))) return GA_E_BADARG;
    if (d->mode == 1 && (!d->p || d->ldq < 2 * d->NL || d->q_rep > 1 || (d->backward && (!d->dmu_q || !d->dp)))) return GA_E_BADARG;
    if (d->mode != 0 && d->mode != 1) return GA_E_UNSUPPORTED;
    if (d->alpha_rows && (d->mode != 0 || d->alpha_col < 0 || d->alpha_ld < 2 * d->alpha_col + 2)) return GA_E_BADARG;
    const long total = (long)d->N * d->h * d->w * d->NL;
    hipLaunchKernelGGL(sampler_kernel, dim3(grid_for(total)), dim3(256), 0, (hipStream_t)s, *d, total);
    return check_launch();
}

extern "C" int ga_dml_mean(const ga_dml_desc* d, void* s) {
    ga::clear_stale_error();
    if (!d || !d->logits || d->N <= 0 || d->H <= 0 || d->W <= 0 || d->nmix <= 0) return GA_E_BADARG;
    if (d->nmix > DML_MAXMIX) return GA_E_UNSUPPORTED;
    if (d->ld < d->nmix * 10 || (d->ld_img != 0 && d->ld_img < 3)) return GA_E_BADARG;
    if (!d->backward && !d->img_nchw && !d->img_nhwc) return GA_E_BADARG;
    if (d->backward && (!d->dlogits || (!d->dimg_nhwc && !d->dimg_nchw))) return GA_E_BADARG;
    if (d->act_rep > 1 && (!d->backward || d->N % d->act_rep)) return GA_E_BADARG;
    const long npix = (long)d->N * d->H * d->W;
    const size_t lds = (size_t)DML_ROWS * (d->ld + 1) * sizeof(float);
    if (lds > 64 * 1024) return GA_E_UNSUPPORTED;
    long blocks = (npix + DML_ROWS - 1) / DML_ROWS;
    if (blocks > 4096) blocks = 4096;
    hipLaunchKernelGGL(dml_kernel, dim3((unsigned)blocks), dim3(DML_ROWS), lds, (hipStream_t)s, *d, npix);
    return check_launch();
}

extern "C" int ga_maxpool2(const ga_maxpool2_desc* d, void* s) {
    ga::clear_stale_error();
    if (!d || !d->x || d->N <= 0 || d->H <= 0 || d->W <= 0 || d->C <= 0) return GA_E_BADARG;
    if ((d->H | d->W) & 1) return GA_E_UNSUPPORTED;
    if (d->C % 4) return GA_E_UNSUPPORTED;
    if (!d->backward && !d->y) return GA_E_BADARG;
    if (d->backward && (!d->dy || !d->dx)) return GA_E_BADARG;
    if (d->act_rep > 1 && (!d->backward || d->N % d->act_rep)) return GA_E_BADARG;
    const long total4 = (long)d->N * (d->H / 2) * (d->W / 2) * (d->C / 4);
    hipLaunchKernelGGL(maxpool2_kernel, dim3(grid_for(total4)), dim3(256), 0, (hipStream_t)s, *d, total4);
    return check_launch();
}

extern "C" int ga_maxpool3s2(const ga_maxpool3s2_desc* d, void* s) {
    ga::clear_stale_error();
    if (!d || !d->x || d->N <= 0 || d->H <= 0 || d->W <= 0 || d->C <= 0) return GA_E_BADARG;
    if (((d->H | d->W) & 1) || (d->C % 4)) return GA_E_UNSUPPORTED;
    if (!d->backward && !d->y) return GA_E_BADARG;
    if (d->backward && (!d->dy || !d->dx)) return GA_E_BADARG;
    const long total4 = d->backward ? (long)d->N * d->H * d->W * (d->C / 4) : (long)d->N * (d->H / 2) * (d->W / 2) * (d->C / 4);
    hipLaunchKernelGGL(maxpool3s2_kernel, dim3(grid_for(total4)), dim3(256), 0, (hipStream_t)s, *d, total4);
    return check_launch();
}

extern "C" int ga_unary(const ga_unary_desc* d, void* s) {
    ga::clear_stale_error();
    if (!d || !d->x || !d->y || d->n <= 0 || d->mode < 0 || d->mode > 3) return GA_E_BADARG;
    if ((d->mode == 1 || d->mode == 3) && !d->g) return GA_E_BADARG;
    hipLaunchKernelGGL(unary_kernel, dim3(grid_for(d->n)), dim3(256), 0, (hipStream_t)s, *d);
    return check_launch();
}

extern "C" int ga_modout(const ga_modout_desc* d, void* s) {
    ga::clear_stale_error();
    if (!d || (!d->t && !d->t_planes[0]) || d->N <= 0 || d->P <= 0 || d->C <= 0) return GA_E_BADARG;
    if (d->C % 4) return GA_E_UNSUPPORTED;
    if (!d->backward && !d->out) return GA_E_BADARG;
    if (d->backward && (!d->dout || (!d->dt && !d->dt_planes[0]))) return GA_E_BADARG;
    if ((d->backward && d->dt_planes[0]) || d->t_planes[0]) {
        if (d->backward && d->dt_planes[0] && (!d->dt_planes[1] || !d->dt_planes[2] || !d->dt_planes[3])) return GA_E_BADARG;
        if (d->t_planes[0] && (!d->t_planes[1] || !d->t_planes[2] || !d->t_planes[3])) return GA_E_BADARG;
        if (d->W <= 0 || d->W % 2 || d->P % d->W || (d->P / d->W) % 2) return GA_E_BADARG;
        if (d->ld_planes % 4) return GA_E_UNSUPPORTED;
        for (int i = 0; i < 4; ++i)
            if ((d->t_planes[0] && !aligned16(d->t_planes[i])) || (d->backward && d->dt_planes[0] && !aligned16(d->dt_planes[i]))) return GA_E_ALIGN;
    }
    if (d->backward && d->red) {
        if (!d->ws || d->ws_floats < (long)d->N * d->C) return GA_E_BADARG;
        if (!aligned16(d->ws) || (d->t && !aligned16(d->t)) || !aligned16(d->dout) || (d->dt && !aligned16(d->dt))) return GA_E_ALIGN;
        const int nchunks = (d->C + 63) / 64;
        long S = d->ws_floats / ((long)d->N * d->C);
        const long want = (2048 + (long)d->N * nchunks - 1) / ((long)d->N * nchunks);
        if (S > want) S = want;
        if (S > (d->P + 255) / 256) S = (d->P + 255) / 256;
        if (S < 1) S = 1;
        const int q = d->C >= 64 ? 16 : d->C / 4;
        int ql = 1;
        while (ql < q) ql <<= 1;
        const int seg_len = (int)((d->P + S - 1) / S);
        hipLaunchKernelGGL(modout_bwd_reduce_kernel, dim3((unsigned)(d->N * nchunks * S)), dim3(256), 0, (hipStream_t)s, *d, nchunks, ql,
                           (int)S, seg_len);
        ga_rowchan_reduce_desc r = {};
        r.out = d->red; r.N = d->N; r.P = d->P; r.C = d->C; r.scale = 1.0f; r.ws = d->ws; r.ws_floats = d->ws_floats;
        const long total = (long)d->N * d->C;
        hipLaunchKernelGGL(rowchan_reduce_final_kernel, dim3((unsigned)((total + 255) / 256)), dim3(256), 0, (hipStream_t)s, r, (int)S);
        return check_launch();
    }
    const long total4 = (long)d->N * d->P * (d->C / 4);
    hipLaunchKernelGGL(modout_kernel, dim3(grid_for(total4)), dim3(256), 0, (hipStream_t)s, *d, total4);
    return check_launch();
}

extern "C" int ga_up2_blur(const ga_up2_blur_desc* d, void* s) {
    ga::clear_stale_error();
    if (!d || d->N <= 0 || d->H <= 0 || d->W <= 0 || d->C <= 0) return GA_E_BADARG;
    if (d->C % 4) return GA_E_UNSUPPORTED;
    if (!d->backward && (!d->lo_in || !d->hi)) return GA_E_BADARG;
    if (d->backward && (!d->hi_in || !d->lo)) return GA_E_BADARG;
    const long total4 = (long)d->N * d->H * d->W * (d->C / 4) * (d->backward ? 1 : 4);
    hipLaunchKernelGGL(up2_blur_kernel, dim3(grid_for(total4)), dim3(256), 0, (hipStream_t)s, *d, total4);
    return check_launch();
}

extern "C" int ga_pixelnorm(const float* x, float* y, long rows, int C, void* s) {
    ga::clear_stale_error();
    if (!x || !y || rows <= 0 || C <= 0) return GA_E_BADARG;
    const long blocks = (rows + 3) / 4;
    hipLaunchKernelGGL(pixelnorm_kernel, dim3((unsigned)(blocks > 65535 ? 65535 : blocks)), dim3(256), 0, (hipStream_t)s, x, y, rows, C);
    return check_launch();
// ... 141 lines not shown
```

### gen_adversarial_amd/engine.py

```python
from __future__ import annotations

import ctypes as C
import json
import os
from typing import Dict, List, Optional, Sequence

import torch

from . import _lib as L
from . import folding as F
from .nvae_spec import DecCellSpec, EncCellSpec, NVAESpec, build_spec
from .e4e_spec import E4ESpec
from .resnet_spec import ResNetSpec
from .vgg_spec import VggSpec
from .engine_core import (IMG_LD, RES_SCALE, TUNE_FILE, WS_FLOATS, Act, WeightStore, _ptr, conv_key,
                          frag_ok, halo_ok, thin_ok, tune_cache)
from .engine_classifiers import ClassifierBuilder
from .engine_e4e import E4EBuilder
from .engine_avae import AvaeBuilder
from .engine_ndvae import NdvaeBuilder
from .engine_nvae import NvaeBuilder
from .engine_stylegan import StyleGanBuilder
from .engine_trans import TransBuilder


def expand_alpha_rows(alphas, rows: int, rep: int, pairs: bool) -> torch.Tensor:
    t = alphas.detach().to('cpu', torch.float64) if isinstance(alphas, torch.Tensor) else torch.tensor(alphas, dtype=torch.float64)
    if t.dim() != 2:
        raise ValueError(f'a [K, n] table of alpha vectors expected, got shape {tuple(t.shape)}')
    K = t.shape[0]
    if K != rows:
        if K < 1 or rep % K or rows % rep:
            raise ValueError(f'{K} candidates do not divide the {rep} rows per image')
        t = t.repeat_interleave(rep // K, dim=0).repeat(rows // rep, 1)
    if not pairs:
        return t.to(torch.float32)
    return torch.stack([t.to(torch.float32), (1.0 - t).to(torch.float32)], dim=2).reshape(rows, -1)


class Engine(NvaeBuilder, NdvaeBuilder, AvaeBuilder, ClassifierBuilder, E4EBuilder, StyleGanBuilder, TransBuilder):
    fuse_dec_cells = os.environ.get('GA_FUSE_DEC_CELL', '1') != '0'
    fuse_min_workgroups = 0 if os.environ.get('GA_FUSE_DEC_CELL') == 'force' else 160
    fuse_halo_cells = os.environ.get('GA_FUSE_HALO_CELL', '0') == '1'
    dec_cell_variant = int(os.environ.get('GA_DEC_CELL_VARIANT', '1'))

    def __init__(self, nvae_sd, nvae_cfg: dict, resolution, vgg_sd, vgg_spec: VggSpec, rows: int, rep: int,
                 alphas: Sequence[float], temperature: float = 0.6, noise_eps: float = 0.0,
                 device: str = 'cuda:0', need_backward: bool = True, dry_run: bool = False,
                 store: Optional[WeightStore] = None, precision: str = 'bf16x3', blur: bool = False,
                 share_encoder: bool = False, cot_rep: int = 1, alpha_rows: bool = False):
        if rows % rep:
            raise ValueError('rows must be a multiple of the EoT repeat')
        self.device = torch.device(device)
        self.dry_run = dry_run
        if self.device.type != 'cuda' and not dry_run:
            raise RuntimeError('the HIP engine needs a GPU device; there is no CPU fallback '
                               '(dry_run=True only builds and validates the plans)')
        if precision not in ('fp32', 'bf16x3'):
            raise ValueError("precision must be 'fp32' (exact f32 MFMA) or 'bf16x3' (3 bf16 MFMAs per product)")
        self.precision = precision
        self.store = store if store is not None else WeightStore(self.device)
        self.has_nvae = nvae_sd is not None
        self.spec: Optional[NVAESpec] = build_spec(nvae_cfg, resolution) if self.has_nvae else None
        self.resolution = tuple(resolution)
        self.vspec = vgg_spec
        self.rows, self.rep = rows, rep
        self.alphas = [float(a) for a in alphas]
        if self.has_nvae and len(self.alphas) != len(self.spec.groups):
            raise ValueError(f'{len(self.spec.groups)} interpolation alphas expected, got {len(self.alphas)}')
        self.temperature = float(temperature)
        self.noise_eps = float(noise_eps)
        self.blur = bool(blur)
        self._init_alpha_rows(alpha_rows)
        self.share_encoder = bool(share_encoder) and rep > 1 and self.noise_eps == 0.0 and nvae_sd is not None
        self.enc_rows = rows // rep if self.share_encoder else rows
        self.need_backward = need_backward
        if cot_rep < 1 or (cot_rep > 1 and not (self.has_nvae or isinstance(vgg_spec, VggSpec))):
            raise ValueError('cot_rep > 1 (K-cotangent backward) is built for the NVAE + VGG defender and the VGG classifier')
        self.cot_rep = int(cot_rep)
        self.bytes = 0
        self.acts = {}
        self.version = 0
        self._sampler_descs = []
        self._keep = []
        self._frag_ok = {}
        self._thin_ok = {}
        self.fwd = L.Plan()
        self.bwd = L.Plan()
        self._bwd_steps = []
        self._build(nvae_sd, vgg_sd)

    @classmethod
    def bare(cls, rows: int, device='cuda:0', precision: str = 'bf16x3', store: Optional[WeightStore] = None,
             dry_run: bool = False, rep: int = 1, resolution=None, alphas: Sequence[float] = (), noise_eps: float = 0.0,
             need_backward: bool = True, blur: bool = False, share_encoder: bool = False, alpha_rows: bool = False) -> "Engine":
        self = cls.__new__(cls)
        self.device, self.dry_run, self.precision = torch.device(device), dry_run, precision
        if self.device.type != 'cuda' and not dry_run:
            raise RuntimeError('the HIP engine needs a GPU device; there is no CPU fallback')
        self.store = store if store is not None else WeightStore(self.device)
        if rows % rep:
            raise ValueError('rows must be a multiple of the EoT repeat')
        self.has_nvae, self.spec, self.vspec, self.resolution = False, None, None, (tuple(resolution) if resolution else None)
        self.rows, self.rep, self.alphas, self.temperature = rows, rep, [float(a) for a in alphas], 1.0
        self.noise_eps, self.blur = float(noise_eps), bool(blur)
        self._init_alpha_rows(alpha_rows)
        self.share_encoder = bool(share_encoder) and rep > 1 and self.noise_eps == 0.0
        self.enc_rows = rows // rep if self.share_encoder else rows
        self.need_backward, self.image_s2d, self.cot_rep = need_backward, False, 1
        self.bytes, self.acts, self.version, self._sampler_descs, self._keep, self._frag_ok, self._thin_ok = 0, {}, 0, [], [], {}, {}
        self.fwd, self.bwd, self._bwd_steps, self._scratch = L.Plan(), L.Plan(), [], {}
        self.eps, self.purified, self.dpurified, self._purified_grad_nhwc = [], None, None, None
        return self

    def finish(self):
        self._finish(0)
        return self

    def _init_alpha_rows(self, alpha_rows: bool):
        self.alpha_rows, self.alpha_table = bool(alpha_rows), None
        if self.alpha_rows and self.rep > 1 and self.noise_eps != 0.0:
            raise ValueError('a per-row alpha engine with rep > 1 shares the encoder pass of an image between its rows: '
                             'not available with input noise (initial_noise_eps > 0)')

    def _alloc_alpha_table(self, n: int, pairs: bool) -> torch.Tensor:
        self._alpha_pairs = pairs
        self.alpha_table = self.alloc((self.rows, (2 if pairs else 1) * n))
        self.alpha_table.copy_(expand_alpha_rows([self.alphas], self.rows, self.rows, pairs))
        return self.alpha_table

    def alloc(self, shape) -> torch.Tensor:
        t = torch.zeros(shape, dtype=torch.float32, device=self.device)
        self.bytes += t.numel() * 4
        self._keep.append(t)
        return t

    def dev(self, t: torch.Tensor) -> torch.Tensor:
        t = t.to(self.device, dtype=torch.float32).contiguous()
        self._keep.append(t)
        self.bytes += t.numel() * 4
        return t

    def devd(self, key: str, fn) -> dict:
        return self.store.get(key, fn)

    def conv(self, plan, name, x, w, y, *, cin=None, cout=None, bias=None, K=1, sn=1, sd=1, pad=0,
             x2=None, pro_scale=None, pro_shift=None, pro_act=0, pro_per_row=0,
             addend=None, addend_bcast=False, addend2=None, dact_x=None, dact_scale=None, dact_shift=None, dact_act=0,
             in_hw=None, out_hw=None, n=None, KH=None, KW=None, anchored=False, explicit_out=False,
             ldx=None, ldy=None, ldadd=None, flags=0, precise=False):
        d = L.ConvDesc()
        N, Hi, Wi, Cx = x.shape
        d.x, d.ldx = _ptr(x), (ldx or Cx)
        d.C1 = cin if cin is not None else Cx
        if x2 is not None:
            d.x2, d.ldx2, d.C2 = _ptr(x2), x2.shape[3], x2.shape[3]
        d.w, d.bias = _ptr(w), _ptr(bias)
        if self.precision == 'bf16x3' and not self.dry_run and not precise:
            hi, lo = self.store.split(w)
            d.w_hi, d.w_lo = _ptr(hi), _ptr(lo)
            kh, kw = (KH or K), (KW or K)
            if (kh, kw, sn, sd, pad) == (3, 3, 1, 1, 1) and x2 is None and (cin or x.shape[3]) % 32 == 0 and 128 % x.shape[2] == 0 \
                    and w.dim() == 2 and w.shape[1] == 9 * (cin or x.shape[3]):
                self._frag_ok[id(d)] = w
            if (kh, kw, sn, sd, pad) == (3, 3, 1, 1, 1) and x2 is None and (cin or x.shape[3]) in (32, 64) and x.shape[1] % 8 == 0 \
                    and x.shape[2] % 16 == 0 and w.dim() == 2 and w.shape[1] == 9 * (cin or x.shape[3]):
                self._thin_ok[id(d)] = w
        d.pro_scale, d.pro_shift, d.pro_act, d.pro_per_row = _ptr(pro_scale), _ptr(pro_shift), pro_act, pro_per_row
        No, Ho, Wo, Cy = y.shape
        d.y, d.ldy = _ptr(y), (ldy or Cy)
        d.flags = flags
        d.Cout = cout if cout is not None else Cy
        if addend is not None:
            d.addend, d.ldadd, d.addend_bcast_n = _ptr(addend), (ldadd or addend.shape[-1]), int(addend_bcast)
        if addend2 is not None:
            d.addend2, d.ldadd2 = _ptr(addend2), addend2.shape[-1]
        if dact_x is not None:
            d.dact_x, d.lddact = _ptr(dact_x), dact_x.shape[-1]
            d.dact_scale, d.dact_shift, d.dact_act = _ptr(dact_scale), _ptr(dact_shift), dact_act
            if dact_x.shape[0] != x.shape[0]:
                assert dact_x.shape[0] * self.cot_rep == x.shape[0], (name, tuple(dact_x.shape), tuple(x.shape), self.cot_rep)
                d.dact_rep = self.cot_rep
        d.N, d.Hi, d.Wi, d.Ho, d.Wo = N, Hi, Wi, Ho, Wo
        d.KH, d.KW = (KH or K), (KW or K)
        d.sn, d.sd, d.pad = sn, sd, pad
        assert No == N, (name, x.shape, y.shape)
        assert w.numel() == d.Cout * d.KH * d.KW * (d.C1 + d.C2), (name, tuple(w.shape), d.Cout, d.KH, d.KW, d.C1, d.C2)
        if anchored:
            assert (Ho, Wo) == (Hi, Wi) and pad == 0 and sn == 1 and sd == 1, name
        elif explicit_out:
            assert (Ho, Wo) == (Hi, Wi) and sn == 1 and sd == 1, name
        elif sd == 1:
            assert (Hi + 2 * pad - K) // sn + 1 == Ho, (name, Hi, Ho, K, sn, pad)
        else:
            assert Ho in (Hi * sd, Hi * sd - 1) or K == 1, (name, Hi, Ho)
        plan.add(d, name)
        return d

    def grad_conv(self, name, x, w, target: Act, *, primary=None, **kw):
        addend, addend2 = primary, None
        if target.g_written:
            if addend is None:
                addend = target.g
            else:
                addend2 = target.g
        d = self.conv(self.bwd, name, x, w, target.g, addend=addend, addend2=addend2, **kw)
        target.g_written = True
        return d

    def gconv(self, plan, name, x, w, y, cg, *, KH=3, KW=3, stride=1, pad=1, bias=None, pro_act=0, dact_x=None, dact_act=0):
        d = L.GconvDesc()
        n, hi, wi, c = x.shape
        _, ho, wo, cy = y.shape
        assert cy == c and c % cg == 0 and w.numel() == c * KH * KW * cg, (name, tuple(x.shape), tuple(y.shape), tuple(w.shape), cg)
        d.x, d.w, d.bias, d.dact_x, d.y = _ptr(x), _ptr(w), _ptr(bias), _ptr(dact_x), _ptr(y)
        d.N, d.Hi, d.Wi, d.Ho, d.Wo, d.C, d.cg = n, hi, wi, ho, wo, c, cg
        d.KH, d.KW, d.stride, d.pad, d.pro_act, d.dact_act = KH, KW, stride, pad, pro_act, dact_act
        plan.add(d, name)
        return d

    def grad_conv_up2(self, name, x, wts, key, target: Act, *, dact_x=None, dact_scale=None, dact_shift=None, dact_act=0, cg=0,
                      dact_prelu=False, ldx=None, **pro):
        n, h, w, _ = x.shape
        il = L.Interleave2Desc()
        for a in (0, 1):
            for b in (0, 1):
                wm = wts.get(f'{key}{a}{b}')
                if wm is None:
                    continue
                taps = wm.shape[1] // (cg or x.shape[3])
                assert taps in (1, 2, 4), (name, tuple(wm.shape), tuple(x.shape))
                kh, kw = 1 + (a if taps >= 2 else 0), 1 + (b if taps >= 2 else 0)
                plane = self.scratch((n, h, w, target.c), f'subpix{a}{b}')
                if cg:
                    self.gconv(self.bwd, f'{name}[{a}{b}]', x, wm, plane, cg, KH=kh, KW=kw, stride=1, pad=0)
                else:
                    self.conv(self.bwd, f'{name}[{a}{b}]', x, wm, plane, KH=kh, KW=kw, pad=0, anchored=True, ldx=ldx, **pro)
                il.s[2 * a + b] = _ptr(plane)
        il.y, il.N, il.H, il.W, il.C = _ptr(target.g), n, 2 * h, 2 * w, target.c
        il.dact_x, il.dact_scale, il.dact_shift, il.dact_act = _ptr(dact_x), _ptr(dact_scale), _ptr(dact_shift), dact_act
        il.dact_prelu = int(dact_prelu)
        if dact_x is not None and dact_x.shape[0] != n:
            assert dact_x.shape[0] * self.cot_rep == n, (name, tuple(dact_x.shape), n)
            il.dact_rep = self.cot_rep
        if target.g_written:
            il.addend = _ptr(target.g)
        self.bwd.add(il, name + '.interleave')
        target.g_written = True

    SE_FUSED_MERGE_MAX = 16384

    def se_forward(self, name, t: Act, wts, P, res_scale=None, merge=None):
        n, c = t.n, t.c
        hd = wts['se_w1'].shape[0]
        hid = self.alloc((n, hd))
        gate = self.alloc((n, c))
        if not hasattr(self, 'small_kinks'):
            self.small_kinks = []
        self.small_kinks.append(hid)
        e = L.SeExciteDesc()
        if merge is None and self._se_wide_rows(n, P, c):
            m = self.alloc((n, c))
            self._se_reduce(self.fwd, f'{name}.se_squeeze', t.t, None, m, n, P, c, 1.0 / P)
            e.m = _ptr(m)
        else:
            e.t = _ptr(t.t)
        e.w1, e.b1, e.w2, e.b2 = _ptr(wts['se_w1']), _ptr(wts['se_b1']), _ptr(wts['se_w2']), _ptr(wts['se_b2'])
        e.hid, e.gate, e.N, e.C, e.Hd, e.P, e.res_scale, e.backward = (_ptr(hid), _ptr(gate), n, c, hd, P,
                                                                        RES_SCALE if res_scale is None else res_scale, 0)
        if merge is not None:
            e.skip, e.out = _ptr(merge[0]), _ptr(merge[1])
        self.fwd.add(e, f'{name}.se_gate' + ('+merge' if merge is not None else ''))
        return gate, hid

    @staticmethod
    def _se_wide_rows(n, P, c) -> bool:
        return n <= 128 and P >= 1024 and P * c >= 262144 and c % 4 == 0

    def _se_reduce(self, plan, name, a, b, out, n, P, c, scale):
        r = L.ReduceDesc()
        r.a, r.b, r.out, r.N, r.P, r.C, r.scale = _ptr(a), _ptr(b), _ptr(out), n, P, c, scale
        ws = self.scratch((256 * n * c,), 'se_reduce_ws')
        r.ws, r.ws_floats = _ptr(ws), ws.numel()
        plan.add(r, name)

    def se_merges(self, t: Act, P) -> bool:
        return P * t.c <= self.SE_FUSED_MERGE_MAX and t.c % 4 == 0

    def se_backward(self, name, dout: torch.Tensor, t: Act, wts, gate, hid, P, res_scale=None):
        n, c = dout.shape[0], t.c
        ps = self.scratch((n, c), f'ps{c}')
        pb = self.scratch((n, c), f'pb{c}')
        e = L.SeExciteDesc()
        rs = RES_SCALE if res_scale is None else res_scale
        if self.cot_rep == 1 and self._se_wide_rows(n, P, c):
            dg = self.scratch((n, c), f'se_dgate{c}')
            self._se_reduce(self.bwd, f'{name}.se_dgate', t.t, dout, dg, n, P, c, rs)
            e.dgate = _ptr(dg)
        else:
            e.act_rep = self.cot_rep
            e.t, e.dout = _ptr(t.t), _ptr(dout)
        e.w1, e.b1, e.w2, e.b2 = _ptr(wts['se_w1']), _ptr(wts['se_b1']), _ptr(wts['se_w2']), _ptr(wts['se_b2'])
        e.hid, e.gate, e.pro_scale, e.pro_shift = _ptr(hid), _ptr(gate), _ptr(ps), _ptr(pb)
        e.N, e.C, e.Hd, e.P, e.res_scale, e.backward = n, c, wts['se_w1'].shape[0], P, (RES_SCALE if res_scale is None else res_scale), 1
        self.bwd.add(e, f'{name}.se_gate_bwd')
        return ps, pb

    def scratch(self, shape, key) -> torch.Tensor:
        k = (key, tuple(shape))
        if k not in self._scratch:
            self._scratch[k] = self.alloc(shape)
        return self._scratch[k]

    def _build(self, nvae_sd, vgg_sd):
        self.nvae_sd = nvae_sd
        self._scratch = {}
        self.image_s2d = (not self.has_nvae) and isinstance(self.vspec, ResNetSpec)
        x0 = self._build_input()
        img = self._build_nvae(x0) if self.has_nvae else x0

        n_nvae_steps = len(self._bwd_steps)
        build = (self._build_resnet if isinstance(self.vspec, ResNetSpec) else
                 self._build_e4e if isinstance(self.vspec, E4ESpec) else self._build_vgg)
        self.logits = build(vgg_sd, img)

        self._finish(n_nvae_steps)

    def _build_input(self) -> Act:
        R = self.rows
        H = self.resolution[1]

        self.x_in = self.alloc((R // self.rep, 3, H, H))
        self.noise = self.alloc((R, 3, H, H)) if self.noise_eps != 0.0 else None
        self.noise_coef = self.alloc((R,)) if self.noise_eps != 0.0 else None
        self.dx = self.alloc((R // self.rep * self.cot_rep, 3, H, H))
        self.eps, self.purified, self.dpurified, self._purified_grad_nhwc = [], None, None, None

        x_src, dx_dst = self.x_in, self.dx
        if self.blur:
            import math
            k = int(2 ** (math.sqrt(H) // 2) - 1)
            xs = torch.arange(k, dtype=torch.float64) - (k - 1) / 2.0
            g = torch.exp(-xs.pow(2) / 2.0)
            taps = self.devd(f'blur_taps_{k}', lambda: {'g': (g / g.sum()).float()})['g']
            x_src = self.alloc((R // self.rep, 3, H, H))
            dx_dst = self.alloc((R // self.rep * self.cot_rep, 3, H, H))
            tmp = self.alloc((R // self.rep, 3, H, H)) if (2 * H * H + k) * 4 > 64 * 1024 else None
            bl = L.BlurDesc()
            bl.x, bl.y, bl.taps, bl.planes, bl.H, bl.W, bl.k, bl.backward = _ptr(self.x_in), _ptr(x_src), _ptr(taps), (R // self.rep) * 3, H, H, k, 0
            bl.radius, bl.tmp = min(12, k // 2), _ptr(tmp)
            self.fwd.add(bl, 'gauss_blur')

            def bwd_blur():
                b = L.BlurDesc()
                b.x, b.y, b.taps, b.planes, b.H, b.W, b.k, b.backward = (_ptr(dx_dst), _ptr(self.dx), _ptr(taps),
                                                                         (R // self.rep) * self.cot_rep * 3, H, H, k, 1)
                b.radius, b.tmp = min(12, k // 2), _ptr(tmp)
                self.bwd.add(b, 'gauss_blur^T')
            self._bwd_steps.append(bwd_blur)

        R0 = self.enc_rows
        rep0 = 1 if self.share_encoder else self.rep
        x0 = Act(self, R0, H // 2, H // 2, 4 * IMG_LD, 'x0') if self.image_s2d else Act(self, R0, H, H, IMG_LD, 'x0')
        io = L.ImageIoDesc()
        io.x_nchw, io.noise_nchw, io.noise_coef, io.y_nhwc = _ptr(x_src), _ptr(self.noise), _ptr(self.noise_coef), _ptr(x0.t)
        io.N, io.C, io.H, io.W, io.rep, io.backward, io.ld, io.s2d = R0, 3, H, H, rep0, 0, IMG_LD, int(self.image_s2d)
        self.fwd.add(io, 'image_in')

        def bwd_image():
            b = L.ImageIoDesc()
            b.x_nchw, b.noise_nchw, b.noise_coef = _ptr(x_src), _ptr(self.noise), _ptr(self.noise_coef)
            b.dy_nhwc, b.dx_nchw = _ptr(x0.g), _ptr(dx_dst)
            b.N, b.C, b.H, b.W, b.rep, b.backward, b.ld, b.s2d = R0 * self.cot_rep, 3, H, H, rep0, 1, IMG_LD, int(self.image_s2d)
            b.cot_rep = self.cot_rep
            self.bwd.add(b, 'image_in^T')
        self._bwd_steps.append(bwd_image)

        return x0

    def _finish(self, n_nvae_steps: int = 0):
        self.bwd_split = 0
        if self.need_backward:
            for step in reversed(self._bwd_steps[n_nvae_steps:]):
                step()
            self.bwd_split = len(self.bwd)
            for step in reversed(self._bwd_steps[:n_nvae_steps]):
                step()
        self._bwd_steps = None
        self.bpda = None
        pg = self._purified_grad_nhwc
        if self.need_backward and pg is not None:
            s2d = int(pg.c == 4 * IMG_LD)
            hp = pg.h * (2 if s2d else 1)
            if hp == self.resolution[1]:
                b = L.ImageIoDesc()
                b.x_nchw, b.dy_nhwc, b.dx_nchw = _ptr(self.x_in), _ptr(pg.g), _ptr(self.dx)
                b.N, b.C, b.H, b.W, b.rep, b.backward, b.ld, b.s2d = self.rows * self.cot_rep, 3, hp, hp, self.rep, 1, IMG_LD, s2d
                b.cot_rep = self.cot_rep
                self.bpda = L.Plan()
                self.bpda.add(b, 'bpda_identity^T')
                self.bpda.finalize()
        self.ws = self.alloc((WS_FLOATS,)) if not self.dry_run else None
        self.apply_tuning(tune_cache())

    def _conv_descs(self):
        return [d for plan in (self.fwd, self.bwd) for d in plan.descs if isinstance(d, L.ConvDesc)]

    def apply_tuning(self, cache: dict):
        for d in self._conv_descs():
            ent = cache.get(conv_key(d), (0, 1, 1))
            tile, splits = ent[0], ent[1]
            use_bf3 = ent[2] if len(ent) > 2 else 1
            need = splits * d.N * d.Ho * d.Wo * d.Cout
            if splits > 1 and (self.ws is None or need > WS_FLOATS):
                tile, splits = 0, 1
            if not use_bf3:
                d.w_hi, d.w_lo = None, None
            if tile == 8 and not (self._want_frag(d) and frag_ok(d, splits)):
                tile = 5
            if tile == 11 and (splits > 1 or not (self._want_thin(d) and thin_ok(d, splits))):
                tile, splits = 7, 1
            if tile in (5, 6, 7) and not halo_ok(d, tile, splits):
                tile, splits = 0, 1
            d.tile, d.splits = int(tile), int(splits)
            d.ws, d.ws_floats = (_ptr(self.ws), WS_FLOATS) if splits > 1 else (None, 0)
        self.fwd.finalize()
        self.bwd.finalize()

    def _want_frag(self, d) -> bool:
        w = self._frag_ok.get(id(d))
        if w is None or self.dry_run:
            return False
        d.w_frag = _ptr(self.store.frag3(w))
        return True

    def _want_thin(self, d) -> bool:
        w = self._thin_ok.get(id(d))
        if w is None or self.dry_run:
            return False
        d.w_frag = _ptr(self.store.frag_thin(w))
        return True

    def autotune(self, cache: Optional[dict] = None, reps: int = 3, save: Optional[str] = None, verbose: bool = False) -> dict:
        if self.dry_run:
            raise RuntimeError('autotune needs a GPU')
        cache = tune_cache() if cache is None else cache
        stream = self.stream()
        for d in self._conv_descs():
            key = conv_key(d)
            if key in cache:
                continue
            M = d.N * d.Ho * d.Wo
            T = d.KH * d.KW * ((d.C1 + d.C2 + 31) // 32)
            best = None
            modes = (1, 0) if d.w_hi else (0,)
            halo = (5, 6, 7) if (d.w_hi and d.KH == 3 and d.KW == 3 and d.sn == 1 and d.sd == 1 and d.C2 == 0) else ()
            if halo and self._want_frag(d):
                halo = halo + (8,)
            thin = (11,) if (d.w_hi and id(d) in self._thin_ok) else ()
            for use_bf3, tile in [(m_, t_) for m_ in modes for t_ in (1, 2, 3, 4) + ((halo + thin) if m_ else ())]:
                bm, bn = {1: (128, 128), 2: (128, 64), 3: (64, 64), 4: (128, 32), 5: (128, 128), 6: (128, 64), 7: (128, 32), 8: (128, 128),
                          11: (128, 32)}[tile]
                if bn >= 2 * max(32, d.Cout) and tile not in (4, 7):
                    continue
                blocks = -(-M // bm) * -(-d.Cout // bn)
                for splits in (1, 2, 4, 8, 16, 32):
                    if splits > 1 and (blocks * splits > 2048 or T < 2 * splits or splits * M * d.Cout > WS_FLOATS):
                        continue
                    if tile >= 5 and splits > d.C1 // 32:
                        continue
                    if tile == 11 and splits > 1:
                        continue
                    t = L.ConvDesc.from_buffer_copy(d)
                    t.tile, t.splits = tile, splits
                    if tile == 11:
                        t.w_frag = _ptr(self.store.frag_thin(self._thin_ok[id(d)]))
                    elif tile == 8:
                        t.w_frag = _ptr(self.store.frag3(self._frag_ok[id(d)]))
                    if not use_bf3:
                        t.w_hi, t.w_lo = None, None
                    t.ws, t.ws_floats = (_ptr(self.ws), WS_FLOATS) if splits > 1 else (None, 0)
                    try:
                        L.run(t, stream)
                    except L.GaError:
                        continue
                    e0, e1 = torch.cuda.Event(enable_timing=True), torch.cuda.Event(enable_timing=True)
                    e0.record()
                    for _ in range(reps):
                        L.run(t, stream)
                    e1.record()
                    e1.synchronize()
                    ms = e0.elapsed_time(e1) / reps
                    if best is None or ms < best[0]:
                        best = (ms, tile, splits, use_bf3)
            cache[key] = (best[1], best[2], best[3])
            if verbose:
                print(f'tune {key}: tile {best[1]} splits {best[2]} {best[0] * 1e3:.1f} us bf3 {best[3]}', flush=True)
        self.apply_tuning(cache)
        if save:
            with open(save, 'w') as f:
                json.dump(cache, f, indent=0, sort_keys=True)
        return cache

    def set_alphas(self, alphas: Sequence[float]):
        alphas = [float(a) for a in alphas]
        if len(alphas) != len(self.alphas):
            raise ValueError(f'{len(self.alphas)} interpolation alphas expected, got {len(alphas)}')
        if self.alpha_table is not None:
            self.alphas = alphas
            self.alpha_table.copy_(expand_alpha_rows([alphas], self.rows, self.rows, self._alpha_pairs))
            return
        if alphas == self.alphas:
            return
        self.alphas = alphas
        if getattr(self, 'alpha_dev', None) is not None:
            self.alpha_dev.copy_(torch.tensor(alphas, dtype=torch.float32))
            return
        for d, idx in self._sampler_descs:
            d.alpha, d.one_minus_alpha = alphas[idx], 1.0 - alphas[idx]
        self.fwd.finalize()
        self.bwd.finalize()
        if getattr(self, '_g_fwd', None) is not None:
            self.enable_graphs()

    def set_alpha_rows(self, alphas):
        if self.alpha_table is None:
            raise RuntimeError('engine was built without a per-row alpha table (alpha_rows=True)')
        t = torch.as_tensor(alphas).detach().to('cpu', torch.float64) if isinstance(alphas, torch.Tensor) else torch.tensor(alphas, dtype=torch.float64)
        if t.dim() != 2 or t.shape[1] != len(self.alphas):
            raise ValueError(f'[K, {len(self.alphas)}] interpolation alphas expected, got {tuple(t.shape)}')
        self.alpha_table.copy_(expand_alpha_rows(t, self.rows, self.rep, self._alpha_pairs))

    def stream(self) -> int:
        return torch.cuda.current_stream(self.device).cuda_stream

    def input_image_nchw(self) -> torch.Tensor:
        t = self.acts['x0'].t
        if not self.image_s2d:
            return t[..., :3].permute(0, 3, 1, 2).contiguous()
        n, h2, w2, _ = t.shape
        v = t.view(n, h2, w2, 2, 2, IMG_LD)[..., :3]
        return v.permute(0, 5, 1, 3, 2, 4).reshape(n, 3, 2 * h2, 2 * w2).contiguous()

    def enable_graphs(self):
        if self.dry_run:
            raise RuntimeError('dry-run engine')
        self.disable_graphs()
        self._side = torch.cuda.Stream(device=self.device)
        cur = torch.cuda.current_stream(self.device)
        self.fwd.run(cur.cuda_stream)
        if self.need_backward:
            self.bwd.run(cur.cuda_stream)
        self._side.wait_stream(cur)
        self._g_fwd = self.fwd.capture(self._side.cuda_stream)
        self._g_bwd = self.bwd.capture(self._side.cuda_stream) if self.need_backward else None
        cur.wait_stream(self._side)

    def disable_graphs(self):
        for h in (getattr(self, '_g_fwd', None), getattr(self, '_g_bwd', None)):
            if h is not None:
                L.Plan.destroy_graph(h)
        self._g_fwd = self._g_bwd = None

    def _launch_graph(self, handle):
        cur = torch.cuda.current_stream(self.device)
        self._side.wait_stream(cur)
        L.Plan.launch_graph(handle, self._side.cuda_stream)
        cur.wait_stream(self._side)

    def forward(self):
        if self.dry_run:
            raise RuntimeError('dry-run engine: plans were built for validation only')
        if getattr(self, '_g_fwd', None) is not None:
            self._launch_graph(self._g_fwd)
        else:
            self.fwd.run(self.stream())

    def backward(self, from_logits: bool = True, from_purified: bool = False, identity_purifier: bool = False):
# ... 26 lines not shown
```

### gen_adversarial_amd/engine_core.py

```python
from __future__ import annotations

import json
import os
from typing import Dict, Optional

import torch

RES_SCALE = 0.1
IMG_LD = 8
WS_FLOATS = 32 * 1024 * 1024
TUNE_FILE = os.path.join(os.path.dirname(os.path.abspath(__file__)), 'conv_tune_gfx950.json')
_TUNE_CACHE: Optional[dict] = None


def tune_cache() -> dict:
    global _TUNE_CACHE
    if _TUNE_CACHE is None:
        _TUNE_CACHE = {}
        if os.path.exists(TUNE_FILE):
            with open(TUNE_FILE) as f:
                _TUNE_CACHE = json.load(f)
    return _TUNE_CACHE


def conv_key(d) -> str:
    return ('b3_' if d.w_hi else '') + '_'.join(str(int(v)) for v in (
        d.N * d.Ho * d.Wo, d.Cout, d.C1, d.C2, d.KH, d.sn, d.sd, d.Hi, d.pro_act, bool(d.pro_scale), d.pro_per_row,
        bool(d.dact_x), d.dact_act, bool(d.addend), bool(d.addend2), d.addend_bcast_n)) + (
        f'_kw{d.KW}' if d.KW != d.KH else '')


def _ptr(t: Optional[torch.Tensor]):
    return None if t is None else t.data_ptr()


_HALO_HK, _HALO_LDH = 32, 40
_BF3_MODES = (0x000, 0x100, 0x001, 0x002, 0x003, 0x004, 0x010, 0x011, 0x020, 0x021)
_HALO_MODES = (0x00, 0x01, 0x02, 0x03, 0x04, 0x10, 0x11, 0x20)


def _a16(p) -> bool:
    return not p or p % 16 == 0


def _pro_mode(d) -> int:
    return ((2 if d.pro_per_row else 1) if d.pro_scale else 0) << 4 | d.pro_act


def _splits(d, splits=None) -> int:
    s = d.splits if splits is None else splits
    if s <= 1:
        return 1
    return min(s, d.KH * d.KW * ((d.C1 + d.C2 + 31) // 32))


def _bf3_vec_out(d, splits: int) -> bool:
    c2 = d.C2 > 0
    vec = d.C1 % 4 == 0 and d.C2 % 4 == 0 and d.ldx % 4 == 0 and (not c2 or d.ldx2 % 4 == 0) and _a16(d.x) and _a16(d.w) \
        and (not c2 or _a16(d.x2)) and (not d.pro_scale or (_a16(d.pro_scale) and _a16(d.pro_shift)))
    bf3 = bool(d.w_hi and d.w_lo) and vec and d.sd == 1 and (not c2 or d.C1 % 32 == 0) and (d.C1 + d.C2) % 8 == 0 \
        and d.KH * d.KW <= 32 and _a16(d.w_hi) and _a16(d.w_lo) and ((0x100 if c2 else 0) | _pro_mode(d)) in _BF3_MODES
    vec_out = d.Cout % 4 == 0 and d.ldy % 4 == 0 and _a16(d.y) and _a16(d.bias) \
        and (not d.addend or (d.ldadd % 4 == 0 and _a16(d.addend))) and (not d.addend2 or (d.ldadd2 % 4 == 0 and _a16(d.addend2))) \
        and (not d.dact_x or (d.lddact % 4 == 0 and _a16(d.dact_x) and (not d.dact_scale or (_a16(d.dact_scale) and _a16(d.dact_shift))))) \
        and (splits == 1 or _a16(d.ws))
    return bf3 and vec_out


def _halo_3x3(d) -> bool:
    if (d.KH, d.KW, d.sn, d.sd, d.pad, d.C2) != (3, 3, 1, 1, 1, 0) or d.Ho != d.Hi or d.Wo != d.Wi or d.C1 % _HALO_HK:
        return False
    howo = d.Ho * d.Wo
    rows = d.Wo < 128 and 128 % d.Wo == 0 and (howo % 128 == 0 or 128 % howo == 0)
    return (rows or d.Wo % 128 == 0) and _pro_mode(d) in _HALO_MODES


def _halo_geometry(d, bm: int = 128, ldh: int = _HALO_LDH):
    howo = d.Ho * d.Wo
    wide = d.Wo >= bm
    tw = bm if wide else d.Wo
    th = 1 if wide else (bm // d.Wo if howo >= bm else d.Ho)
    ni = 1 if howo >= bm else bm // howo
    ph, pw = th + 2, tw + 2

    def pad_to(nbytes, want):
        return nbytes + ((want - nbytes) % 256 + 256) % 256
    rs = pad_to(pw * ldh * 2, (tw * ldh * 2) % 256)
    is_ = pad_to(ph * rs, (th * tw * ldh * 2) % 256) // 2
    return ni, ni * ph * pw, is_


def halo_ok(d, tile: Optional[int] = None, splits: Optional[int] = None) -> bool:
    tile = d.tile if tile is None else tile
    s = _splits(d, splits)
    if tile not in (5, 6, 7) or not _bf3_vec_out(d, s) or not _halo_3x3(d):
        return False
    ni, p, is_ = _halo_geometry(d)
    if p > 13 * 32 or (p > 9 * 32 and _pro_mode(d) not in (0x00, 0x10, 0x20)) or s > d.C1 // _HALO_HK:
        return False
    bn = {5: 128, 6: 64, 7: 32}[tile]
    return (2 * ni * is_ + 2 * 2 * bn * _HALO_LDH) * 2 <= 160 * 1024


def frag_ok(d, splits: Optional[int] = None) -> bool:
    s = _splits(d, splits)
    if not d.w_frag or not _a16(d.w_frag) or not _bf3_vec_out(d, s) or not _halo_3x3(d):
        return False
    ni, p, is_ = _halo_geometry(d)
    if p > 9 * 32 or s > d.C1 // _HALO_HK:
        return False
    mode = _pro_mode(d)
    patch = 2 * ni * is_ * 2
    rp = (p * 8 + 255) >> 8
    tab = rp * 256 * 6 + (2 * (ni if mode == 0x20 else 1) * d.C1 * 4 if mode >= 0x10 else 0)
    dbuf = 2 * patch + tab <= 80 * 1024
    tab_off = ((2 if dbuf else 1) * patch + 15) // 16 * 4
    return tab_off * 4 + tab <= 80 * 1024


def thin_ok(d, splits: Optional[int] = None) -> bool:
    s = _splits(d, splits)
    if s != 1 or not d.w_frag or not _a16(d.w_frag) or not _bf3_vec_out(d, s):
        return False
    if (d.KH, d.KW, d.sn, d.sd, d.pad, d.C2) != (3, 3, 1, 1, 1, 0) or d.C1 not in (32, 64):
        return False
    return d.Ho == d.Hi and d.Wo == d.Wi and d.Ho % 8 == 0 and d.Wo % 16 == 0 and d.Wo <= 255 * 16 and _pro_mode(d) in _HALO_MODES


class WeightStore:

    def __init__(self, device):
        self.device = torch.device(device)
        self.cache: Dict[str, dict] = {}
        self.splits: Dict[int, tuple] = {}
        self.bytes = 0

    def split(self, w: torch.Tensor):
        k = w.data_ptr()
        if k not in self.splits:
            hi = w.to(torch.bfloat16)
            lo = (w - hi.float()).to(torch.bfloat16)
            self.splits[k] = (hi.contiguous(), lo.contiguous(), w)
            self.bytes += 4 * w.numel()
        return self.splits[k][0], self.splits[k][1]

    def frag3(self, w: torch.Tensor, m16: bool = False) -> torch.Tensor:
        k = ('frag3m16' if m16 else 'frag3', w.data_ptr())
        if k not in self.splits:
            hi, lo = self.split(w)
            cout, kk = w.shape
            c = kk // 9
            nt, nkc = (cout + 127) // 128, c // 32

            def arr(t):
                tp = torch.zeros(nt * 128, kk, dtype=torch.bfloat16, device=t.device)
                tp[:cout] = t
                if m16:
                    return tp.view(nt, 4, 2, 16, 9, nkc, 4, 8).permute(0, 5, 4, 1, 2, 6, 3, 7)
                return tp.view(nt, 4, 32, 9, nkc, 2, 2, 8).permute(0, 4, 3, 1, 5, 6, 2, 7)
            f = torch.stack([arr(hi), arr(lo)], dim=5).contiguous()
            self.splits[k] = (f, w)
            self.bytes += 2 * f.numel()
        return self.splits[k][0]

    def frag_thin(self, w: torch.Tensor) -> torch.Tensor:
        k = ('frag_thin', w.data_ptr())
        if k not in self.splits:
            hi, lo = self.split(w)
            cout, kk = w.shape
            assert kk in (9 * 32, 9 * 64), tuple(w.shape)
            nt, ks = (cout + 31) // 32, kk // 9 // 16

            def arr(t):
                tp = torch.zeros(nt * 32, kk, dtype=torch.bfloat16, device=t.device)
                tp[:cout] = t
                return tp.view(nt, 32, 9, ks, 2, 8).permute(0, 2, 3, 4, 1, 5)
            f = torch.stack([arr(hi), arr(lo)], dim=3).contiguous()
            self.splits[k] = (f, w)
            self.bytes += 2 * f.numel()
        return self.splits[k][0]

    def get(self, key: str, fn):
        if key not in self.cache:
            d = {k: v.to(self.device, dtype=torch.float32).contiguous() for k, v in fn().items()}
            self.bytes += sum(v.numel() * 4 for v in d.values())
            self.cache[key] = d
        return self.cache[key]


class Act:

    def __init__(self, eng: "Engine", n, h, w, c, name=''):
        self.eng, self.n, self.h, self.w, self.c, self.name = eng, n, h, w, c, name
        self.t = eng.alloc((n, h, w, c))
        self._g = None
        self.g_written = False
        eng.acts[name] = self

    @property
    def g(self) -> torch.Tensor:
        if self._g is None:
            self._g = self.eng.alloc((self.n * getattr(self.eng, 'cot_rep', 1), self.h, self.w, self.c))
        return self._g
```

### gen_adversarial_amd/engine_nvae.py

```python
from __future__ import annotations

from typing import Dict, Optional

import torch

from . import _lib as L
from . import folding as F
from .engine_core import IMG_LD, RES_SCALE, Act, _ptr
from .ndvae_spec import NdGenCell, NdResCell
from .nvae_spec import DecCellSpec, EncCellSpec


class NvaeBuilder:
    def enc_cell(self, cell: EncCellSpec, x: Act) -> Act:
        nd = isinstance(cell, NdResCell)
        wts = self.devd(('nd.' if nd else '') + cell.prefix, lambda: (F.fold_nd_res_cell if nd else F.fold_enc_cell)(self.nvae_sd, cell))
        rs = getattr(cell, 'res_scale', RES_SCALE)
        n, h, w = x.n, x.h, x.w
        st = 2 if cell.down else 1
        ho, wo = h // st, w // st
        t1 = Act(self, n, ho, wo, cell.cout, cell.prefix + '.t1')
        t2 = Act(self, n, ho, wo, cell.cout, cell.prefix + '.t2')
        out = Act(self, n, ho, wo, cell.cout, cell.prefix + '.out')
        p = cell.prefix
        self.conv(self.fwd, p + '.conv1', x.t, wts['w1'], t1.t, bias=wts['b1'], K=3, sn=st, pad=1,
                  pro_scale=wts['pro_scale'], pro_shift=wts['pro_shift'], pro_act=L.GA_ACT_SILU)
        self.conv(self.fwd, p + '.conv2', t1.t, wts['w2'], t2.t, bias=wts['b2'], K=3, pad=1, pro_act=L.GA_ACT_SILU)
        if cell.down:
            sk = Act(self, n, ho, wo, cell.cout, p + '.skip')
            ks = 2 if wts['ws'].shape[1] == 4 * x.c else 1
            self.conv(self.fwd, p + '.skip', x.t, wts['ws'], sk.t, bias=wts['bs'], K=ks, sn=2, pad=0, pro_act=L.GA_ACT_SILU)
            skip_t = sk.t
        else:
            skip_t = x.t
        if self.se_merges(t2, ho * wo):
            gate, hid = self.se_forward(p, t2, wts, ho * wo, res_scale=rs, merge=(skip_t, out.t))
        else:
            gate, hid = self.se_forward(p, t2, wts, ho * wo, res_scale=rs)
            a = L.SeApplyDesc()
            a.skip, a.t, a.gate, a.out = _ptr(skip_t), _ptr(t2.t), _ptr(gate), _ptr(out.t)
            a.N, a.H, a.W, a.C, a.skip_mode, a.res_scale = n, ho, wo, cell.cout, 0, rs
            self.fwd.add(a, p + '.merge')

        def backward():
            ps, pb = self.se_backward(p, out.g, t2, wts, gate, hid, ho * wo, res_scale=rs)
            dt1 = self.scratch((out.g.shape[0], ho, wo, cell.cout), 'enc_dt1')
            self.conv(self.bwd, p + '.conv2^T', out.g, wts['w2_bwd'], dt1, K=3, pad=1,
                      pro_scale=ps, pro_shift=pb, pro_per_row=1, dact_x=t1.t, dact_act=L.GA_ACT_SILU)
            if cell.down:
                self.grad_conv_up2(p + '.conv1^T', dt1, wts, 'w1_sub', x, dact_x=x.t, dact_scale=wts['pro_scale'],
                                   dact_shift=wts['pro_shift'], dact_act=L.GA_ACT_SILU)
                self.grad_conv_up2(p + '.skip^T', out.g, wts, 'ws_sub', x, dact_x=x.t, dact_act=L.GA_ACT_SILU)
            else:
                self.grad_conv(p + '.conv1^T', dt1, wts['w1_bwd'], x, K=3, sn=1, sd=1, pad=1, primary=out.g,
                               dact_x=x.t, dact_scale=wts['pro_scale'], dact_shift=wts['pro_shift'], dact_act=L.GA_ACT_SILU)
        self._bwd_steps.append(backward)
        return out

    def dec_cell(self, cell: DecCellSpec, x: Act) -> Act:
        nd = isinstance(cell, NdGenCell)
        wts = self.devd(('nd.' if nd else '') + cell.prefix, lambda: (F.fold_nd_gen_cell if nd else F.fold_dec_cell)(self.nvae_sd, cell))
        rs = getattr(cell, 'res_scale', RES_SCALE)
        n, h, w = x.n, x.h, x.w
        up = cell.up
        H, W = (2 * h, 2 * w) if up else (h, w)
        hid_c = cell.hidden
        p = cell.prefix
        fused = (not up and not nd and self.precision == 'bf16x3' and self.fuse_dec_cells and cell.cout == x.c
                 and L.lib.ga_dec_cell_supported(n, H, W, x.c, hid_c) == 1
                 and n * H * W // (256 if x.c == 128 else 128) >= self.fuse_min_workgroups)
        halo = (not fused and not up and not nd and self.precision == 'bf16x3' and self.fuse_dec_cells
                and (self.fuse_halo_cells or not self.need_backward) and cell.cout == x.c
                and self.cot_rep == 1 and L.lib.ga_dec_cell_halo_supported(n, H, W, x.c, hid_c) == 1
                and n * H * W // 128 >= self.fuse_min_workgroups)
        t3 = Act(self, n, H, W, cell.cout, p + '.t3')
        out = Act(self, n, H, W, cell.cout, p + '.out')

        def halo_desc(backward: int) -> L.DecCellHaloDesc:
            f = L.DecCellHaloDesc()
            f.x, f.b1, f.wd, f.wd_bwd, f.bd, f.b2 = (_ptr(x.t), _ptr(wts['b1']), _ptr(wts['wd']), _ptr(wts['wd_bwd']),
                                                    _ptr(wts['bd']), _ptr(wts['b2']))
            if not self.dry_run:
                (h1, l1), (h2, l2) = self.store.split(wts['w1']), self.store.split(wts['w2_bwd' if backward else 'w2'])
                f.w1_hi, f.w1_lo, f.w2_hi, f.w2_lo = _ptr(h1), _ptr(l1), _ptr(h2), _ptr(l2)
                if backward:
                    h3, l3 = self.store.split(wts['w1_bwd'])
                    f.w1t_hi, f.w1t_lo = _ptr(h3), _ptr(l3)
            f.N, f.H, f.W, f.Cin, f.Cout, f.Hd, f.backward, f.up = n, H, W, x.c, cell.cout, hid_c, backward, 0
            return f

        def fused_desc(backward: int) -> L.DecCellDesc:
            f = L.DecCellDesc()
            f.x, f.b1, f.wd, f.wd_bwd, f.bd, f.b2 = (_ptr(x.t), _ptr(wts['b1']), _ptr(wts['wd']), _ptr(wts['wd_bwd']),
                                                    _ptr(wts['bd']), _ptr(wts['b2']))
            if not self.dry_run:
                (h1, l1), (h2, l2) = self.store.split(wts['w1']), self.store.split(wts['w2_bwd' if backward else 'w2'])
                f.w1_hi, f.w1_lo, f.w2_hi, f.w2_lo = _ptr(h1), _ptr(l1), _ptr(h2), _ptr(l2)
            f.N, f.H, f.W, f.C, f.Hd, f.backward = n, H, W, x.c, hid_c, backward
            f.variant = self.dec_cell_variant if x.c == 128 else 0
            return f

        if fused:
            f = fused_desc(0)
            f.y = _ptr(t3.t)
            self.fwd.add(f, p + '.cell')
        elif halo:
            f = halo_desc(0)
            f.y = _ptr(t3.t)
            self.fwd.add(f, p + '.cell')
        else:
            t1 = Act(self, n, h, w, hid_c, p + '.t1')
            t2 = Act(self, n, H, W, hid_c, p + '.t2')
            self.conv(self.fwd, p + '.pw1', x.t, wts['w1'], t1.t, bias=wts['b1'], K=1)
            d = L.DwDesc()
            d.x, d.w, d.bias, d.y = _ptr(t1.t), _ptr(wts['wd']), _ptr(wts['bd']), _ptr(t2.t)
            d.N, d.H, d.W, d.C, d.pro_act, d.up2 = n, H, W, hid_c, L.GA_ACT_SILU, int(up)
            self.fwd.add(d, p + '.dw5')
            if nd:
                u = t2
                t2 = Act(self, n, H, W, hid_c, p + '.t2p')
                self.conv(self.fwd, p + '.pw', u.t, wts['wp'], t2.t, bias=wts['bp'], K=1)
            self.conv(self.fwd, p + '.pw2', t2.t, wts['w2'], t3.t, bias=wts['b2'], K=1, pro_act=L.GA_ACT_SILU)
        if not up and self.se_merges(t3, H * W):
            gate, hid = self.se_forward(p, t3, wts, H * W, res_scale=rs, merge=(x.t, out.t))
        else:
            a = L.SeApplyDesc()
            if up:
                sl = Act(self, n, h, w, cell.cout, p + '.skip_low')
                self.conv(self.fwd, p + '.skip', x.t, wts['ws'], sl.t, bias=wts['bs'], K=1)
                a.skip, a.skip_mode = _ptr(sl.t), 1
            else:
                a.skip, a.skip_mode = _ptr(x.t), 0
            gate, hid = self.se_forward(p, t3, wts, H * W, res_scale=rs)
            a.t, a.gate, a.out = _ptr(t3.t), _ptr(gate), _ptr(out.t)
            a.N, a.H, a.W, a.C, a.res_scale = n, H, W, cell.cout, rs
            self.fwd.add(a, p + '.merge')

        def backward():
            nc = out.g.shape[0]
            ps, pb = self.se_backward(p, out.g, t3, wts, gate, hid, H * W, res_scale=rs)
            if halo:
                b = halo_desc(1)
                b.dout, b.pro_scale, b.pro_shift, b.addend, b.y = _ptr(out.g), _ptr(ps), _ptr(pb), _ptr(out.g), _ptr(x.g)
                if x.g_written:
                    b.addend2 = _ptr(x.g)
                self.bwd.add(b, p + '.cell^T')
                x.g_written = True
                return
            dt1 = self.scratch((nc, h, w, hid_c), 'dec_dt1')
            if fused:
                b = fused_desc(1)
                b.dout, b.pro_scale, b.pro_shift, b.y = _ptr(out.g), _ptr(ps), _ptr(pb), _ptr(dt1)
                b.N, b.act_rep = nc, self.cot_rep
                self.bwd.add(b, p + '.cell^T')
            else:
                dt2 = self.scratch((nc, H, W, hid_c), 'dec_dt2')
                self.conv(self.bwd, p + '.pw2^T', out.g, wts['w2_bwd'], dt2, K=1,
                          pro_scale=ps, pro_shift=pb, pro_per_row=1, dact_x=t2.t, dact_act=L.GA_ACT_SILU)
                if nd:
                    du = self.scratch((nc, H, W, hid_c), 'dec_du')
                    self.conv(self.bwd, p + '.pw^T', dt2, wts['wp_bwd'], du, K=1)
                    dt2 = du
                b = L.DwDesc()
                b.x, b.w, b.dact_x, b.y = _ptr(dt2), _ptr(wts['wd_bwd']), _ptr(t1.t), _ptr(dt1)
                b.N, b.H, b.W, b.C, b.dact_act, b.pool2, b.act_rep = nc, H, W, hid_c, L.GA_ACT_SILU, int(up), self.cot_rep
                self.bwd.add(b, p + '.dw5^T')
            self.grad_conv(p + '.pw1^T', dt1, wts['w1_bwd'], x, K=1, primary=None if up else out.g)
            if up:
                dsl = self.scratch((nc, h, w, cell.cout), 'dec_dsl')
                bl = L.BilinearBwdDesc()
                bl.dhigh, bl.dlow, bl.N, bl.h, bl.w, bl.C, bl.accumulate = _ptr(out.g), _ptr(dsl), nc, h, w, cell.cout, 0
                self.bwd.add(bl, p + '.bilinear^T')
                self.grad_conv(p + '.skip^T', dsl, wts['ws_bwd'], x, K=1)
        self._bwd_steps.append(backward)
        return out

    def _build_nvae(self, x0: Act) -> Act:
        nvae_sd = self.nvae_sd
        spec, R = self.spec, self.rows
        H = spec.resolution
        NL = spec.num_latent
        self.latent_pitch = (NL + 7) // 8 * 8
        self.eps = [self.alloc((R, NL, gs.res, gs.res)) for gs in spec.groups]
        self.purified = self.alloc((R, 3, H, H))
        if self.alpha_rows:
            self._alloc_alpha_table(len(spec.groups), pairs=True)

        stem = self.devd('stem', lambda: F.pad_image_conv(F.fold_wn_conv(nvae_sd, 'preprocessing_block.init_conv'), 3, IMG_LD))
        norm = self.devd('norm05', lambda: {'two': torch.full((IMG_LD,), 2.0), 'mone': torch.full((IMG_LD,), -1.0)})
        two, mone = norm['two'], norm['mone']
        RE = self.enc_rows
        erep = self.rep if self.share_encoder else 1
        x = Act(self, RE, H, H, spec.base_channels, 'stem')
        self.conv(self.fwd, 'stem', x0.t, stem['w'], x.t, bias=stem['b'], K=3, pad=1, pro_scale=two, pro_shift=mone)
        stem_out = x

        def bwd_stem():
            self.grad_conv('stem^T', stem_out.g, stem['w_bwd'], x0, K=3, pad=1,
                           dact_x=x0.t, dact_scale=two, dact_shift=mone, dact_act=L.GA_ACT_NONE)
        self._bwd_steps.append(bwd_stem)

        for cell in spec.pre_cells:
            x = self.enc_cell(cell, x)

        stash: Dict[str, Act] = {}
        for kind, payload in spec.enc_program:
            if kind == 'stash':
                stash[payload] = x
            else:
                x = self.enc_cell(payload, x)
        x_top = x

        C0 = spec.enc0_channels
        g0 = spec.groups[0]
        enc0 = self.devd('encoder_0', lambda: F.fold_wn_conv(nvae_sd, 'encoder_0.1'))
        e0 = Act(self, RE, g0.res, g0.res, C0, 'enc0')
        self.conv(self.fwd, 'encoder_0', x_top.t, enc0['w'], e0.t, bias=enc0['b'], K=1, pro_act=L.GA_ACT_ELU)
        NLP = self.latent_pitch
        s00 = self.devd('enc_sampler_0:0', lambda: F.pad_conv_out(
            F.fold_wn_conv(nvae_sd, 'enc_sampler.sampler_0:0', out_slice=slice(0, NL)), NL, NLP))
        muq0 = Act(self, RE, g0.res, g0.res, NLP, 'mu_q0')
        self.conv(self.fwd, 'enc_sampler_0:0', e0.t, s00['w'], muq0.t, bias=s00['b'], K=3, pad=1, pro_act=L.GA_ACT_ELU)
        z = Act(self, R, g0.res, g0.res, NLP, 'z0')
        self._sampler_fwd('sample_0:0', muq0, None, self.eps[0], z, self.alphas[0], q_rep=erep)

        def fold_comb0():
            wfull = F.wn_weight64(nvae_sd, 'decoder_combiners.combiner_0:0.conv')[:, :, 0, 0]
            prior = nvae_sd['const_prior'].double()[0]
            pc = torch.einsum('oc,chw->hwo', wfull[:, :C0], prior) + \
                nvae_sd['decoder_combiners.combiner_0:0.conv.bias'].double()
            if spec.num_nf_cells:
                pc = pc - wfull[:, C0:] @ F.nf_constant_shift(nvae_sd, '0:0', spec.num_nf_cells, NL)
            return {'pc': pc.float().unsqueeze(0), 'wz': F.pad_cols(wfull[:, C0:].float(), 0, NL, NLP),
                    'wz_bwd': F.pad_rows(wfull[:, C0:].t().float().contiguous(), NLP)}
        c0w = self.devd('combiner_0:0', fold_comb0)
        pc, wz, wz_bwd = c0w['pc'], c0w['wz'], c0w['wz_bwd']
        x = Act(self, R, g0.res, g0.res, C0, 'comb_0:0')
        self.conv(self.fwd, 'combiner_0:0', z.t, wz, x.t, K=1, addend=pc, addend_bcast=True)
        comb0_out, z0 = x, z

        def bwd_group0():
            self.grad_conv('combiner_0:0^T', comb0_out.g, wz_bwd, z0, K=1)
            self._sampler_bwd('sample_0:0^T', muq0, None, self.eps[0], z0, self.alphas[0], None, q_rep=erep)
            self.grad_conv('enc_sampler_0:0^T', muq0.g, s00['w_bwd'], e0, K=3, pad=1, dact_x=e0.t, dact_act=L.GA_ACT_ELU)
            self.grad_conv('encoder_0^T', e0.g, enc0['w_bwd'], x_top, K=1, dact_x=x_top.t, dact_act=L.GA_ACT_ELU)
        group0_bwd = bwd_group0

        dec_bwd_steps_start = len(self._bwd_steps)
        self._bwd_steps.append(group0_bwd)

        for gs in spec.groups:
            if gs.dec_cells:
                for cell in gs.dec_cells:
                    x = self.dec_cell(cell, x)
                x = self._latent_group(gs, x, stash[f'{gs.s}:{gs.g}'], erep)
            if gs.g == spec.groups_per_scale[gs.s] - 1 and gs.s in spec.dec_up_cells:
                x = self.dec_cell(spec.dec_up_cells[gs.s], x)

        for cell in spec.post_cells:
            x = self.dec_cell(cell, x)

        LO = (spec.logits_out + 7) // 8 * 8
        tl = self.devd('to_logits', lambda: F.pad_conv_out(F.fold_wn_conv(nvae_sd, 'to_logits.1'), spec.logits_out, LO))
        logits = Act(self, R, H, H, LO, 'mix_logits')
        post_out = x
        self.conv(self.fwd, 'to_logits', x.t, tl['w'], logits.t, bias=tl['b'], K=3, pad=1, pro_act=L.GA_ACT_ELU)
        img = Act(self, R, H, H, IMG_LD, 'purified_nhwc')
        dm = L.DmlDesc()
        dm.logits, dm.ld, dm.nmix, dm.img_nchw, dm.img_nhwc = _ptr(logits.t), LO, spec.num_mixtures, _ptr(self.purified), _ptr(img.t)
        dm.N, dm.H, dm.W, dm.backward, dm.ld_img = R, H, H, 0, IMG_LD
        self.fwd.add(dm, 'dml_mean')
        self.dpurified = self.alloc((R * self.cot_rep, 3, H, H))
        purified_img = img

        def bwd_dml():
            b = L.DmlDesc()
            b.logits, b.ld, b.nmix, b.dimg_nhwc, b.dlogits = _ptr(logits.t), LO, spec.num_mixtures, _ptr(img.g), _ptr(logits.g)
            b.dimg_nchw = _ptr(self.dpurified)
            b.N, b.H, b.W, b.backward, b.ld_img, b.act_rep = R * self.cot_rep, H, H, 1, IMG_LD, self.cot_rep
            self.bwd.add(b, 'dml_mean^T')
            self.grad_conv('to_logits^T', logits.g, tl['w_bwd'], post_out, K=3, pad=1, dact_x=post_out.t, dact_act=L.GA_ACT_ELU)
        self._bwd_steps.append(bwd_dml)

        self._purified_grad_nhwc = purified_img
        return img

# ... 112 lines not shown
```

### include/ga_ops.h

```cpp
#ifndef GA_OPS_H
#define GA_OPS_H

#ifdef __cplusplus
extern "C" {
#endif

#define GA_OK            0
#define GA_E_BADARG     -1
#define GA_E_ALIGN      -2
#define GA_E_UNSUPPORTED -3
#define GA_E_LAUNCH     -4

enum ga_act { GA_ACT_NONE = 0, GA_ACT_SILU = 1, GA_ACT_ELU = 2, GA_ACT_RELU = 3,
              GA_ACT_LRELU = 4 ,
              GA_ACT_FLRELU = 5  };
enum ga_conv_flags { GA_CONV_ADDEND_RELU = 1, GA_CONV_ADDEND_PRE_DACT = 2, GA_CONV_PRO_PRELU = 4, GA_CONV_DACT_PRELU = 8 };

typedef struct ga_conv_desc {
    const float* x;          int ldx;
    const float* x2;         int ldx2;
    const float* w;
    const float* bias;
    const float* pro_scale;
    const float* pro_shift;
    const float* addend;     int ldadd;
    const float* addend2;    int ldadd2;
    const float* dact_x;     int lddact;
    const float* dact_scale;
    const float* dact_shift;
    float* y;                int ldy;
    int N, Hi, Wi, C1, C2;
    int Ho, Wo, Cout;
    int KH, KW, sn, sd, pad;
    int pro_act, pro_per_row;
    int dact_act;
    int addend_bcast_n;
    int tile;
    int splits;
    float* ws;
    long ws_floats;
    unsigned x_bytes, x2_bytes, w_bytes;
    int dact_rep;
    const void* w_hi;
    const void* w_lo;
    int addend_rep;
    int flags;
    const void* w_frag;
} ga_conv_desc;
int ga_conv2d(const ga_conv_desc* d, void* stream);

typedef struct ga_dwconv5_desc {
    const float* x;
    const float* w;
    const float* bias;
    const float* dact_x;
    float* y;
    int N, H, W, C;
    int pro_act, dact_act, up2, pool2;
    int act_rep;
    int _reserved;
} ga_dwconv5_desc;
int ga_dwconv5(const ga_dwconv5_desc* d, void* stream);

typedef struct ga_rowchan_reduce_desc {
    const float* a; const float* b; float* out;
    int N, P, C; float scale;
    float* ws; long ws_floats;
    const float* gate; const float* skip; float* scaled;
    const float* a_src; const float* a_w;
} ga_rowchan_reduce_desc;
int ga_rowchan_reduce(const ga_rowchan_reduce_desc* d, void* stream);

typedef struct ga_se_excite_desc {
    const float* m;
    const float* w1; const float* b1;
    const float* w2; const float* b2;
    float* hid;
    float* gate;
    const float* dgate;
    float* pro_scale; float* pro_shift;
    int N, C, Hd, P; float res_scale; int backward;
    const float* t; const float* dout;
    const float* skip; float* out;
    int act_rep; int _reserved;
} ga_se_excite_desc;
int ga_se_excite(const ga_se_excite_desc* d, void* stream);

typedef struct ga_se_apply_desc {
    const float* skip; const float* t; const float* gate; float* out;
    int N, H, W, C; int skip_mode; float res_scale;
} ga_se_apply_desc;
int ga_se_apply(const ga_se_apply_desc* d, void* stream);

typedef struct ga_bilinear_up2_bwd_desc {
    const float* dhigh; float* dlow; int N, h, w, C; int accumulate;
} ga_bilinear_up2_bwd_desc;
int ga_bilinear_up2_bwd(const ga_bilinear_up2_bwd_desc* d, void* stream);

typedef struct ga_sampler_desc {
    const float* mu_q; int ldq;
    const float* p;    int ldp;
    const float* eps;  int eps_nchw;
    float* z;
    const float* dz;
    float* dmu_q; float* dp;
    int N, h, w, NL; float alpha, one_minus_alpha, temp; int backward;
    int q_rep;
    float* dmu_q_rows;
    int ldz;
    int act_rep;
    int mode;
    int _reserved;
    const float* alpha_rows;
    int alpha_ld; int alpha_col;
} ga_sampler_desc;
int ga_sampler_mix(const ga_sampler_desc* d, void* stream);

typedef struct ga_dml_desc {
    const float* logits; int ld; int nmix;
    float* img_nchw; float* img_nhwc;
    const float* dimg_nhwc; const float* dimg_nchw; float* dlogits;
    int N, H, W; int backward;
    int ld_img;
    int act_rep;
} ga_dml_desc;
int ga_dml_mean(const ga_dml_desc* d, void* stream);

typedef struct ga_maxpool2_desc {
    const float* x; float* y; const float* dy; float* dx; int N, H, W, C; int backward;
    int act_rep;
} ga_maxpool2_desc;
int ga_maxpool2(const ga_maxpool2_desc* d, void* stream);

typedef struct ga_gconv_desc {
    const float* x; const float* w; const float* bias; const float* dact_x; float* y;
    int N, Hi, Wi, Ho, Wo, C, cg;
    int KH, KW, stride, pad;
    int pro_act, dact_act;
    int _reserved;
} ga_gconv_desc;
int ga_gconv(const ga_gconv_desc* d, void* stream);

typedef struct ga_unary_desc { const float* x; const float* g; float* y; long n; int mode; float eps; } ga_unary_desc;
int ga_unary(const ga_unary_desc* d, void* stream);

typedef struct ga_modout_desc {
    const float* t; const float* scale; const float* add; float* out; const float* dout; float* dt;
    int N, P, C; int act; int backward;
    int W;
    float* dt_planes[4];
    int ld_planes;
    int _reserved2;
    float* red;
    float* ws; long ws_floats;
    const float* t_planes[4];
} ga_modout_desc;
int ga_modout(const ga_modout_desc* d, void* stream);

typedef struct ga_up2_blur_desc { const float* lo_in; float* hi; const float* hi_in; float* lo; int N, H, W, C; int backward; int _reserved; } ga_up2_blur_desc;
int ga_up2_blur(const ga_up2_blur_desc* d, void* stream);

int ga_pixelnorm(const float* x, float* y, long rows, int C, void* stream);

typedef struct ga_latent_mix_desc {
    const float* codes; const float* avg; const float* styles; const float* alpha; float* out;
    const float* dout; float* dcodes; int R, J, D; int backward;
    int rep;
    int alpha_ld;
} ga_latent_mix_desc;
int ga_latent_mix(const ga_latent_mix_desc* d, void* stream);

typedef struct ga_pool_denorm_desc {
    const float* x; float* y; const float* dy; float* dx; int N, H, W, k, ld; int backward;
    const float* dy_nchw;
    int band;
    int _reserved;
} ga_pool_denorm_desc;
int ga_pool_denorm(const ga_pool_denorm_desc* d, void* stream);

typedef struct ga_attn_desc {
    const float* q; const float* k; const float* v; float* out; float* p;
    const float* dout; float* ds; float* dq; float* dk; float* dv;
    int ldq, ldk, ldv, ldo, lddq, lddk, lddv;
    int N, Tq, Tk, heads, dh;
    float scale;
    int backward;
} ga_attn_desc;
int ga_attn(const ga_attn_desc* d, void* stream);

typedef struct ga_layernorm_desc {
    const float* a; const float* b; const float* gamma; const float* beta; float* y; float* stats;
    const float* dy; float* dx;
    long rows; int C; float eps; int backward; int accumulate;
} ga_layernorm_desc;
int ga_layernorm(const ga_layernorm_desc* d, void* stream);

typedef struct ga_resize2_crop_desc {
    const float* x; float* y; const float* dy; float* dx; int N, H, W, C, crop; int backward; int accumulate; int _reserved;
} ga_resize2_crop_desc;
int ga_resize2_crop(const ga_resize2_crop_desc* d, void* stream);

typedef struct ga_dec_cell_desc {
    const float* x;
    const void* w1_hi; const void* w1_lo; const float* b1;
    const float* wd; const float* wd_bwd; const float* bd;
    const void* w2_hi; const void* w2_lo; const float* b2;
    const float* dout; const float* pro_scale; const float* pro_shift;
    float* y;
    int N, H, W, C, Hd; int backward;
    int act_rep;
    int variant;
} ga_dec_cell_desc;
int ga_dec_cell(const ga_dec_cell_desc* d, void* stream);
int ga_dec_cell_supported(int N, int H, int W, int C, int Hd);

typedef struct ga_dec_cell_halo_desc {
    const float* x;
    const void* w1_hi; const void* w1_lo; const float* b1;
    const float* wd; const float* wd_bwd; const float* bd;
    const void* w2_hi; const void* w2_lo; const float* b2;
    const void* w1t_hi; const void* w1t_lo;
    const float* dout; const float* pro_scale; const float* pro_shift;
    const float* addend; const float* addend2;
    float* y;
    int N, H, W, Cin, Cout, Hd; int backward, up;
} ga_dec_cell_halo_desc;
int ga_dec_cell_halo(const ga_dec_cell_halo_desc* d, void* stream);
int ga_dec_cell_halo_supported(int N, int H, int W, int C, int Hd);

enum { GA_AVAE_ADAIN = 0, GA_AVAE_AVGPOOL = 1, GA_AVAE_PIXELNORM = 2, GA_AVAE_SAMPLE = 3 };
typedef struct ga_avae_desc {
    const float* x; const float* a; const float* b; const float* c; const float* s; const float* dy;
    float* y; float* y2;
    int mode, backward;
    int N, P, C, k, H, W;
    float f0; int _reserved;
} ga_avae_desc;
// ... 107 lines not shown
```

Baseline: 6164 defender rows/s (rows = images x EoT-32).

## Fuse SE squeeze reductions into producing conv epilogue as per-block partial sums

The conv epilogue can now write per-16-row partial channel sums (forward) or partial dot products with the SE input (backward) into a small buffer. The SE excite kernel then reduces those partials instead of re-reading the full activation tensor. Link resolution happens at plan finalisation and is on by default. The aim is to cut a full activation re-read per SE block, at the cost of extra LDS traffic, a syncthreads in the conv epilogue, and an extra strided rdot_t load.

Result: no change. 6152 defender rows/s (rows = images x EoT-32) (-0.2%).

```diff
diff --git a/gen_adversarial_amd/_lib.py b/gen_adversarial_amd/_lib.py
--- a/gen_adversarial_amd/_lib.py
+++ b/gen_adversarial_amd/_lib.py
@@ -15,6 +15,7 @@
  GA_OP_MAXPOOL3S2, GA_OP_AVGPOOL_ACT, GA_OP_GCONV, GA_OP_PRELU, GA_OP_UNARY, GA_OP_MODOUT, GA_OP_UP2_BLUR, GA_OP_PIXELNORM,
  GA_OP_LATENT_MIX, GA_OP_POOL_DENORM, GA_OP_ATTN, GA_OP_LAYERNORM, GA_OP_RESIZE2_CROP, GA_OP_DEC_CELL, GA_OP_AVAE, GA_OP_DEC_CELL_HALO) = range(1, 31)
 GA_AVAE_ADAIN, GA_AVAE_AVGPOOL, GA_AVAE_PIXELNORM, GA_AVAE_SAMPLE = 0, 1, 2, 3
+GA_RED_BLOCK = 16
 ABI_VERSION = 8
 ERRORS = {0: 'GA_OK', -1: 'GA_E_BADARG', -2: 'GA_E_ALIGN', -3: 'GA_E_UNSUPPORTED', -4: 'GA_E_LAUNCH'}
 
@@ -34,7 +35,8 @@
                 ('pro_act', i32), ('pro_per_row', i32), ('dact_act', i32), ('addend_bcast_n', i32), ('tile', i32),
                 ('splits', i32), ('ws', fp), ('ws_floats', C.c_long),
                 ('x_bytes', C.c_uint), ('x2_bytes', C.c_uint), ('w_bytes', C.c_uint), ('dact_rep', i32),
-                ('w_hi', fp), ('w_lo', fp), ('addend_rep', i32), ('flags', i32), ('w_frag', fp)]
+                ('w_hi', fp), ('w_lo', fp), ('addend_rep', i32), ('flags', i32), ('w_frag', fp),
+                ('rsum', C.c_size_t), ('rdot', C.c_size_t), ('rdot_t', C.c_size_t), ('ldrt', i32), ('rdot_rep', i32)]
 
 
 class DwDesc(C.Structure):
@@ -52,7 +54,7 @@
     _fields_ = [('m', fp), ('w1', fp), ('b1', fp), ('w2', fp), ('b2', fp), ('hid', fp), ('gate', fp),
                 ('dgate', fp), ('pro_scale', fp), ('pro_shift', fp),
                 ('N', i32), ('C', i32), ('Hd', i32), ('P', i32), ('res_scale', f32), ('backward', i32),
-                ('t', fp), ('dout', fp), ('skip', fp), ('out', fp), ('act_rep', i32), ('_reserved', i32)]
+                ('t', fp), ('dout', fp), ('skip', fp), ('out', fp), ('act_rep', i32), ('nblk', i32), ('part', fp)]
 
 
 class SeApplyDesc(C.Structure):
@@ -333,6 +335,14 @@
     def __init__(self):
         self.descs = []
         self.names = []
+        self.attached = {}
+        self._arr = None
+
+    def attach(self, desc, **fields):
+        if fields:
+            self.attached[id(desc)] = fields
+        else:
+            self.attached.pop(id(desc), None)
         self._arr = None
 
     def add(self, desc, name: str = ''):
@@ -344,6 +354,8 @@
         arr = (Op * len(self.descs))()
         for i, d in enumerate(self.descs):
             arr[i] = make_op(d)
+            for k, v in self.attached.get(id(d), {}).items():
+                setattr(getattr(arr[i].u, _KIND_FIELD[arr[i].kind]), k, v)
         self._arr = arr
         return self
 
diff --git a/gen_adversarial_amd/csrc/conv_epilogue.h b/gen_adversarial_amd/csrc/conv_epilogue.h
--- a/gen_adversarial_amd/csrc/conv_epilogue.h
+++ b/gen_adversarial_amd/csrc/conv_epilogue.h
@@ -106,7 +106,8 @@
         const int q = tid % QL, rr = tid / QL;
         const int co = n0 + 4 * q;
         const bool mine = co < d.Cout;
-        floatx4 u[1][NB], a1[1][NB], a2[1][NB];
+        floatx4 u[1][NB], a1[1][NB], a2[1][NB], tq[1][NB];
+        float* const red = ws ? nullptr : (d.rsum ? d.rsum : d.rdot);
         auto issue = [&](const int set, const int rb0) __attribute__((always_inline)) {
 #pragma unroll
             for (int k = 0; k < NB; ++k) {
@@ -126,6 +127,11 @@
                 if (d.addend2) {
                     const size_t m = ok ? (size_t)mr : 0;
                     a2[set][k] = *reinterpret_cast<const floatx4*>(d.addend2 + m * d.ldadd2 + co);
+                }
+                if (d.rdot) {
+                    size_t m = ok ? (size_t)mr : 0;
+                    if (d.rdot_rep > 1) m = ((m / HoWo) / d.rdot_rep) * HoWo + (m % HoWo);
+                    tq[set][k] = *reinterpret_cast<const floatx4*>(d.rdot_t + m * d.ldrt + co);
                 }
             }
         };
@@ -188,6 +194,22 @@
                     }
                     if (d.addend2) o += a2[set][k];
                     if (ok[k]) *reinterpret_cast<floatx4*>(d.y + (size_t)mrow(rb0 + k * ROWS) * d.ldy + co) = o;
+                    if (red) *reinterpret_cast<floatx4*>(Cs + (rb0 + k * ROWS) * LDC + 4 * q) = d.rdot ? o * tq[set][k] : o;
+                }
+            }
+        }
+        if (red) {
+            __syncthreads();
+            constexpr int NBLK = BM / 16;
+            for (int task = tid; task < NBLK * QL; task += 256) {
+                const int q2 = task % QL, b = task / QL;
+                const int cq = n0 + 4 * q2, mb = mrow(16 * b);
+                if (cq < d.Cout && mb < M) {
+                    const float* src = Cs + (16 * b) * LDC + 4 * q2;
+                    floatx4 s = *reinterpret_cast<const floatx4*>(src);
+#pragma unroll
+                    for (int i = 1; i < 16; ++i) s += *reinterpret_cast<const floatx4*>(src + i * LDC);
+                    *reinterpret_cast<floatx4*>(red + (size_t)(mb >> 4) * d.Cout + cq) = s;
                 }
             }
         }
diff --git a/gen_adversarial_amd/csrc/conv_mfma.hip b/gen_adversarial_amd/csrc/conv_mfma.hip
--- a/gen_adversarial_amd/csrc/conv_mfma.hip
+++ b/gen_adversarial_amd/csrc/conv_mfma.hip
@@ -420,6 +420,15 @@
     if (d.addend2 && d.ldadd2 < d.Cout) return GA_E_BADARG;
     if (d.dact_x && d.lddact < d.Cout) return GA_E_BADARG;
     if (d.dact_x && d.dact_rep > 1 && d.N % d.dact_rep) return GA_E_BADARG;
+    const bool want_red = d.rsum || d.rdot;
+    if (want_red) {
+        if (d.rsum && d.rdot) return GA_E_UNSUPPORTED;
+        if (d.rdot && (!d.rdot_t || d.ldrt < d.Cout)) return GA_E_BADARG;
+        if (d.rdot && d.rdot_rep > 1 && d.N % d.rdot_rep) return GA_E_BADARG;
+        if (((long)d.Ho * d.Wo) % GA_RED_BLOCK || d.splits > 1) return GA_E_UNSUPPORTED;
+        if (!aligned16(d.rsum ? d.rsum : d.rdot)) return GA_E_ALIGN;
+        if (d.rdot && (!aligned16(d.rdot_t) || d.ldrt % 4)) return GA_E_ALIGN;
+    }
     {
         const long row_x = (long)d.Hi * d.Wi * d.ldx * 4, row_x2 = d.C2 > 0 ? (long)d.Hi * d.Wi * d.ldx2 * 4 : 0;
         long row_max = row_x > row_x2 ? row_x : row_x2;
@@ -430,6 +439,7 @@
         if (d.dact_x && pix_out * d.lddact > row_max) row_max = pix_out * d.lddact;
         const long lim = ga_conv_row_limit();
         if (d.N > 1 && row_max * d.N >= lim && row_max < lim) {
+            if (want_red) return GA_E_UNSUPPORTED;
             int sub = (int)((lim - 1) / row_max);
             const int arep = d.addend && !d.addend_bcast_n && d.addend_rep > 1 ? d.addend_rep : 1;
             const int drep = d.dact_x && d.dact_rep > 1 ? d.dact_rep : 1;
@@ -480,6 +490,7 @@
                                         (!d.dact_scale || (aligned16(d.dact_scale) && aligned16(d.dact_shift))))) &&
                          (splits == 1 || aligned16(d.ws));
 
+    if (want_red && !vec_out) return GA_E_UNSUPPORTED;
     int tile = d.tile;
     if (tile == 0) {
         if (d.Cout <= 32) tile = 4;
diff --git a/gen_adversarial_amd/csrc/elementwise.hip b/gen_adversarial_amd/csrc/elementwise.hip
--- a/gen_adversarial_amd/csrc/elementwise.hip
+++ b/gen_adversarial_amd/csrc/elementwise.hip
@@ -132,18 +132,43 @@
     float* s_part = sm + ((d.C + d.Hd + 3) & ~3);
     const int n = blockIdx.x, tid = threadIdx.x;
     const int na = (d.backward && d.act_rep > 1) ? n / d.act_rep : n;
-    if (d.t) {
+    if (d.part || d.t) {
         const int C4 = d.C >> 2, PL = 256 / C4;
         const int q = tid % C4, pl = tid / C4;
         if (pl < PL) {
             floatx4 acc = {0.f, 0.f, 0.f, 0.f};
             const float* a = d.t + (size_t)na * d.P * d.C + 4 * q;
             const float* b = d.backward ? d.dout + (size_t)n * d.P * d.C + 4 * q : nullptr;
+            if (d.part || d.P % GA_RED_BLOCK == 0) {
+                const int nblk = d.part ? d.nblk : d.P / GA_RED_BLOCK;
+                const int per = (nblk + PL - 1) / PL;
+                const int b0 = pl * per, b1 = min(nblk, b0 + per);
+                if (d.part) {
+                    const float* pp = d.part + (size_t)n * nblk * d.C + 4 * q;
 #pragma unroll 8
-            for (int p = pl; p < d.P; p += PL) {
-                floatx4 v = *reinterpret_cast<const floatx4*>(a + (size_t)p * d.C);
-                if (b) v *= *reinterpret_cast<const floatx4*>(b + (size_t)p * d.C);
-                acc += v;
+                    for (int k = b0; k < b1; ++k) acc += *reinterpret_cast<const floatx4*>(pp + (size_t)k * d.C);
+                } else {
+                    for (int k = b0; k < b1; ++k) {
+                        floatx4 v[GA_RED_BLOCK];
+#pragma unroll
+                        for (int i = 0; i < GA_RED_BLOCK; ++i) {
+                            const size_t o = (size_t)(k * GA_RED_BLOCK + i) * d.C;
+                            v[i] = *reinterpret_cast<const floatx4*>(a + o);
+                            if (b) v[i] *= *reinterpret_cast<const floatx4*>(b + o);
+                        }
+                        floatx4 sb = v[0];
+#pragma unroll
+                        for (int i = 1; i < GA_RED_BLOCK; ++i) sb += v[i];
+                        acc += sb;
+                    }
+                }
+            } else {
+#pragma unroll 8
+                for (int p = pl; p < d.P; p += PL) {
+                    floatx4 v = *reinterpret_cast<const floatx4*>(a + (size_t)p * d.C);
+                    if (b) v *= *reinterpret_cast<const floatx4*>(b + (size_t)p * d.C);
+                    acc += v;
+                }
             }
             *reinterpret_cast<floatx4*>(s_part + pl * d.C + 4 * q) = acc;
         }
@@ -162,7 +187,7 @@
     const int per = (C4 + chunks - 1) / chunks;
     float* s_red = s_part;
     if (!d.backward) {
-        if (!d.t) {
+        if (!d.t && !d.part) {
             for (int c = tid; c < d.C; c += 256) s_in[c] = d.m[(size_t)n * d.C + c];
             __syncthreads();
         }
@@ -184,12 +209,13 @@
         }
         __syncthreads();
         if (tid < d.Hd) {
-            float h = d.b1[tid];
+            float h = 0.f;
             for (int k = 0; k < chunks; ++k) h += s_red[tid * chunks + k];
             if (d.C & 3) {
-                h = d.b1[tid];
+                h = 0.f;
                 for (int c = 0; c < d.C; ++c) h += d.w1[(size_t)tid * d.C + c] * s_in[c];
             }
+            h += d.b1[tid];
             s_hid[tid] = h;
             d.hid[(size_t)n * d.Hd + tid] = h;
         }
@@ -229,7 +255,7 @@
     } else {
         for (int c = tid; c < d.C; c += 256) {
             const float g = d.gate[(size_t)na * d.C + c];
-            const float dg = d.t ? s_in[c] : d.dgate[(size_t)n * d.C + c];
+            const float dg = (d.t || d.part) ? s_in[c] : d.dgate[(size_t)n * d.C + c];
             s_in[c] = dg * g * (1.f - g);
         }
         __syncthreads();
@@ -1169,16 +1195,18 @@
 extern "C" int ga_se_excite(const ga_se_excite_desc* d, void* s) {
     ga::clear_stale_error();
     if (!d || !d->w1 || !d->b1 || !d->w2 || !d->b2 || !d->hid || !d->gate || d->N <= 0 || d->C <= 0 || d->Hd <= 0) return GA_E_BADARG;
-    if (!d->backward && !d->m && !d->t) return GA_E_BADARG;
-    if (d->backward && ((!d->dgate && !d->t) || !d->pro_scale || !d->pro_shift || d->P <= 0)) return GA_E_BADARG;
+    if (!d->backward && !d->m && !d->t && !d->part) return GA_E_BADARG;
+    if (d->backward && ((!d->dgate && !d->t && !d->part) || !d->pro_scale || !d->pro_shift || d->P <= 0)) return GA_E_BADARG;
     if (d->out && (d->backward || !d->t || !aligned16(d->out) || (d->skip && !aligned16(d->skip)))) return GA_E_BADARG;
-    if (d->act_rep > 1 && (!d->backward || !d->t || d->N % d->act_rep)) return GA_E_BADARG;
+    if (d->act_rep > 1 && (!d->backward || (!d->t && !d->part) || d->N % d->act_rep)) return GA_E_BADARG;
+    if (d->part && (d->P <= 0 || d->nblk <= 0 || (long)d->nblk * GA_RED_BLOCK != d->P)) return GA_E_BADARG;
+    if (d->part && d->backward && d->t) return GA_E_BADARG;
     size_t lds = (size_t)(d->C + d->Hd + 4 + 256) * sizeof(float);
     if (d->Hd > 256) return GA_E_UNSUPPORTED;
-    if (d->t) {
-        if (d->P <= 0 || (d->backward && !d->dout)) return GA_E_BADARG;
+    if (d->t || d->part) {
+        if (d->P <= 0 || (d->t && d->backward && !d->dout)) return GA_E_BADARG;
         if (d->C % 4 || d->C > 1024) return GA_E_UNSUPPORTED;
-        if (!aligned16(d->t) || (d->dout && !aligned16(d->dout))) return GA_E_ALIGN;
+        if ((d->t && !aligned16(d->t)) || (d->dout && !aligned16(d->dout)) || (d->part && !aligned16(d->part))) return GA_E_ALIGN;
         const size_t red = (size_t)(256 / (d->C / 4)) * d->C * sizeof(float);
         if (red > 256 * sizeof(float)) lds += red - 256 * sizeof(float);
     }
diff --git a/gen_adversarial_amd/engine.py b/gen_adversarial_amd/engine.py
--- a/gen_adversarial_amd/engine.py
+++ b/gen_adversarial_amd/engine.py
@@ -14,7 +14,7 @@
 from .resnet_spec import ResNetSpec
 from .vgg_spec import VggSpec
 from .engine_core import (IMG_LD, RES_SCALE, TUNE_FILE, WS_FLOATS, Act, WeightStore, _ptr, conv_key,
-                          frag_ok, halo_ok, thin_ok, tune_cache)
+                          frag_ok, halo_ok, reduce_ok, thin_ok, tune_cache)
 from .engine_classifiers import ClassifierBuilder
 from .engine_e4e import E4EBuilder
 from .engine_avae import AvaeBuilder
@@ -43,6 +43,7 @@
     fuse_min_workgroups = 0 if os.environ.get('GA_FUSE_DEC_CELL') == 'force' else 160
     fuse_halo_cells = os.environ.get('GA_FUSE_HALO_CELL', '0') == '1'
     dec_cell_variant = int(os.environ.get('GA_DEC_CELL_VARIANT', '1'))
+    fuse_se_reductions = os.environ.get('GA_FUSE_SE_REDUCE', '1') != '0'
 
     def __init__(self, nvae_sd, nvae_cfg: dict, resolution, vgg_sd, vgg_spec: VggSpec, rows: int, rep: int,
                  alphas: Sequence[float], temperature: float = 0.6, noise_eps: float = 0.0,
@@ -85,6 +86,8 @@
         self._keep = []
         self._frag_ok = {}
         self._thin_ok = {}
+        self._se_links = []
+        self._part_free = {}
         self.fwd = L.Plan()
         self.bwd = L.Plan()
         self._bwd_steps = []
@@ -110,6 +113,7 @@
         self.need_backward, self.image_s2d, self.cot_rep = need_backward, False, 1
         self.bytes, self.acts, self.version, self._sampler_descs, self._keep, self._frag_ok, self._thin_ok = 0, {}, 0, [], [], {}, {}
         self.fwd, self.bwd, self._bwd_steps, self._scratch = L.Plan(), L.Plan(), [], {}
+        self._se_links, self._part_free = [], {}
         self.eps, self.purified, self.dpurified, self._purified_grad_nhwc = [], None, None, None
         return self
 
@@ -250,7 +254,7 @@
 
     SE_FUSED_MERGE_MAX = 16384
 
-    def se_forward(self, name, t: Act, wts, P, res_scale=None, merge=None):
+    def se_forward(self, name, t: Act, wts, P, res_scale=None, merge=None, producer=None):
         n, c = t.n, t.c
         hd = wts['se_w1'].shape[0]
         hid = self.alloc((n, hd))
@@ -265,6 +269,8 @@
             e.m = _ptr(m)
         else:
             e.t = _ptr(t.t)
+            if isinstance(producer, L.ConvDesc) and producer.y == _ptr(t.t):
+                self._link_se_reduction('rsum', self.fwd, producer, e, t.t, None, n, P, c, 1, keep_t=merge is not None)
         e.w1, e.b1, e.w2, e.b2 = _ptr(wts['se_w1']), _ptr(wts['se_b1']), _ptr(wts['se_w2']), _ptr(wts['se_b2'])
         e.hid, e.gate, e.N, e.C, e.Hd, e.P, e.res_scale, e.backward = (_ptr(hid), _ptr(gate), n, c, hd, P,
                                                                         RES_SCALE if res_scale is None else res_scale, 0)
@@ -300,11 +306,57 @@
         else:
             e.act_rep = self.cot_rep
             e.t, e.dout = _ptr(t.t), _ptr(dout)
+            writer = self._last_writer(dout)
+            if writer is not None:
+                self._link_se_reduction('rdot', self.bwd, writer, e, t.t, dout, n, P, c, self.cot_rep)
         e.w1, e.b1, e.w2, e.b2 = _ptr(wts['se_w1']), _ptr(wts['se_b1']), _ptr(wts['se_w2']), _ptr(wts['se_b2'])
         e.hid, e.gate, e.pro_scale, e.pro_shift = _ptr(hid), _ptr(gate), _ptr(ps), _ptr(pb)
         e.N, e.C, e.Hd, e.P, e.res_scale, e.backward = n, c, wts['se_w1'].shape[0], P, (RES_SCALE if res_scale is None else res_scale), 1
         self.bwd.add(e, f'{name}.se_gate_bwd')
         return ps, pb
+
+    def _last_writer(self, g: torch.Tensor, window: int = 16):
+        lo = g.data_ptr()
+        hi = lo + g.numel() * 4
+
+        def touches(d):
+            for f, _ in d._fields_:
+                v = getattr(d, f)
+                for u in (v if isinstance(v, C.Array) else (v,)):
+                    if isinstance(u, int) and not isinstance(u, bool) and lo <= u < hi:
+                        return True
+            return False
+        for d in reversed(self.bwd.descs[-window:]):
+            if touches(d):
+                ok = isinstance(d, L.ConvDesc) and d.y == lo and d.ldy == d.Cout and d.N * d.Ho * d.Wo * d.Cout == g.numel()
+                return d if ok else None
+        return None
+
+    def _link_se_reduction(self, kind, plan, cv, e, t, dout, n, P, c, rep, keep_t=False):
+        if P % L.GA_RED_BLOCK or c % 4 or cv.Cout != c or cv.ldy != c or cv.N * cv.Ho * cv.Wo != n * P \
+                or any(l[2] is cv for l in self._se_links):
+            return
+        part = self.scratch((n, P // L.GA_RED_BLOCK, c), 'se_part_' + kind)
+        at = max(i for i, d in enumerate(plan.descs) if d is cv)
+        if at < self._part_free.get((id(plan), part.data_ptr()), 0):
+            return
+        self._part_free[(id(plan), part.data_ptr())] = len(plan.descs) + 1
+        self._se_links.append((kind, plan, cv, e, dict(part=_ptr(part), nblk=P // L.GA_RED_BLOCK, t=_ptr(t), dout=_ptr(dout), c=c, rep=rep,
+                                                 keep_t=keep_t)))
+
+    def _resolve_se_links(self):
+        for kind, plan, cv, e, a in self._se_links:
+            on = self.fuse_se_reductions and reduce_ok(cv)
+            e.part, e.nblk = (a['part'], a['nblk']) if on else (None, 0)
+            if not on:
+                plan.attach(cv)
+                e.t, e.dout = a['t'], a['dout']
+            elif kind == 'rsum':
+                plan.attach(cv, rsum=a['part'])
+                e.t = a['t'] if a['keep_t'] else None
+            else:
+                plan.attach(cv, rdot=a['part'], rdot_t=a['t'], ldrt=a['c'], rdot_rep=a['rep'])
+                e.t, e.dout = None, None
 
     def scratch(self, shape, key) -> torch.Tensor:
         k = (key, tuple(shape))
@@ -424,6 +476,7 @@
                 tile, splits = 0, 1
             d.tile, d.splits = int(tile), int(splits)
             d.ws, d.ws_floats = (_ptr(self.ws), WS_FLOATS) if splits > 1 else (None, 0)
+        self._resolve_se_links()
         self.fwd.finalize()
         self.bwd.finalize()
 
diff --git a/gen_adversarial_amd/engine_core.py b/gen_adversarial_amd/engine_core.py
--- a/gen_adversarial_amd/engine_core.py
+++ b/gen_adversarial_amd/engine_core.py
@@ -127,6 +127,18 @@
     return d.Ho == d.Hi and d.Wo == d.Wi and d.Ho % 8 == 0 and d.Wo % 16 == 0 and d.Wo <= 255 * 16 and _pro_mode(d) in _HALO_MODES
 
 
+def reduce_ok(d) -> bool:
+    if d.splits > 1 or (d.Ho * d.Wo) % 16:
+        return False
+    vec_out = d.Cout % 4 == 0 and d.ldy % 4 == 0 and _a16(d.y) and _a16(d.bias) \
+        and (not d.addend or (d.ldadd % 4 == 0 and _a16(d.addend))) and (not d.addend2 or (d.ldadd2 % 4 == 0 and _a16(d.addend2))) \
+        and (not d.dact_x or (d.lddact % 4 == 0 and _a16(d.dact_x) and (not d.dact_scale or (_a16(d.dact_scale) and _a16(d.dact_shift)))))
+    row_in = d.Hi * d.Wi * 4 * max(d.ldx, d.ldx2 if d.C2 > 0 else 0)
+    row_out = d.Ho * d.Wo * 4 * max(d.ldy, d.ldadd if d.addend and not d.addend_bcast_n else 0, d.ldadd2 if d.addend2 else 0,
+                                    d.lddact if d.dact_x else 0)
+    return vec_out and max(row_in, row_out) * d.N < 0x7fffff00
+
+
 class WeightStore:
 
     def __init__(self, device):
diff --git a/gen_adversarial_amd/engine_nvae.py b/gen_adversarial_amd/engine_nvae.py
--- a/gen_adversarial_amd/engine_nvae.py
+++ b/gen_adversarial_amd/engine_nvae.py
@@ -25,7 +25,7 @@
         p = cell.prefix
         self.conv(self.fwd, p + '.conv1', x.t, wts['w1'], t1.t, bias=wts['b1'], K=3, sn=st, pad=1,
                   pro_scale=wts['pro_scale'], pro_shift=wts['pro_shift'], pro_act=L.GA_ACT_SILU)
-        self.conv(self.fwd, p + '.conv2', t1.t, wts['w2'], t2.t, bias=wts['b2'], K=3, pad=1, pro_act=L.GA_ACT_SILU)
+        c2 = self.conv(self.fwd, p + '.conv2', t1.t, wts['w2'], t2.t, bias=wts['b2'], K=3, pad=1, pro_act=L.GA_ACT_SILU)
         if cell.down:
             sk = Act(self, n, ho, wo, cell.cout, p + '.skip')
             ks = 2 if wts['ws'].shape[1] == 4 * x.c else 1
@@ -34,9 +34,9 @@
         else:
             skip_t = x.t
         if self.se_merges(t2, ho * wo):
-            gate, hid = self.se_forward(p, t2, wts, ho * wo, res_scale=rs, merge=(skip_t, out.t))
-        else:
-            gate, hid = self.se_forward(p, t2, wts, ho * wo, res_scale=rs)
+            gate, hid = self.se_forward(p, t2, wts, ho * wo, res_scale=rs, merge=(skip_t, out.t), producer=c2)
+        else:
+            gate, hid = self.se_forward(p, t2, wts, ho * wo, res_scale=rs, producer=c2)
             a = L.SeApplyDesc()
             a.skip, a.t, a.gate, a.out = _ptr(skip_t), _ptr(t2.t), _ptr(gate), _ptr(out.t)
             a.N, a.H, a.W, a.C, a.skip_mode, a.res_scale = n, ho, wo, cell.cout, 0, rs
@@ -100,6 +100,7 @@
             f.variant = self.dec_cell_variant if x.c == 128 else 0
             return f
 
+        pw2 = None
         if fused:
             f = fused_desc(0)
             f.y = _ptr(t3.t)
@@ -120,9 +121,9 @@
                 u = t2
                 t2 = Act(self, n, H, W, hid_c, p + '.t2p')
                 self.conv(self.fwd, p + '.pw', u.t, wts['wp'], t2.t, bias=wts['bp'], K=1)
-            self.conv(self.fwd, p + '.pw2', t2.t, wts['w2'], t3.t, bias=wts['b2'], K=1, pro_act=L.GA_ACT_SILU)
+            pw2 = self.conv(self.fwd, p + '.pw2', t2.t, wts['w2'], t3.t, bias=wts['b2'], K=1, pro_act=L.GA_ACT_SILU)
         if not up and self.se_merges(t3, H * W):
-            gate, hid = self.se_forward(p, t3, wts, H * W, res_scale=rs, merge=(x.t, out.t))
+            gate, hid = self.se_forward(p, t3, wts, H * W, res_scale=rs, merge=(x.t, out.t), producer=pw2)
         else:
             a = L.SeApplyDesc()
             if up:
@@ -131,7 +132,7 @@
                 a.skip, a.skip_mode = _ptr(sl.t), 1
             else:
                 a.skip, a.skip_mode = _ptr(x.t), 0
-            gate, hid = self.se_forward(p, t3, wts, H * W, res_scale=rs)
+            gate, hid = self.se_forward(p, t3, wts, H * W, res_scale=rs, producer=pw2)
             a.t, a.gate, a.out = _ptr(t3.t), _ptr(gate), _ptr(out.t)
             a.N, a.H, a.W, a.C, a.res_scale = n, H, W, cell.cout, rs
             self.fwd.add(a, p + '.merge')
diff --git a/include/ga_ops.h b/include/ga_ops.h
--- a/include/ga_ops.h
+++ b/include/ga_ops.h
@@ -46,7 +46,12 @@
     int addend_rep;
     int flags;
     const void* w_frag;
+    float* rsum;
+    float* rdot;
+    const float* rdot_t;     int ldrt;
+    int rdot_rep;
 } ga_conv_desc;
+#define GA_RED_BLOCK 16
 int ga_conv2d(const ga_conv_desc* d, void* stream);
 
 typedef struct ga_dwconv5_desc {
@@ -82,7 +87,9 @@
     int N, C, Hd, P; float res_scale; int backward;
     const float* t; const float* dout;
     const float* skip; float* out;
-    int act_rep; int _reserved;
+    int act_rep;
+    int nblk;
+    const float* part;
 } ga_se_excite_desc;
 int ga_se_excite(const ga_se_excite_desc* d, void* stream);
 
```
